# DmitryUlyanov/deep-image-prior

Hardware: AMD Instinct MI355X
Metric: optimisation iters/sec per image (skip-net 512x512 denoising) (higher is better)
Workload: dtype f32

## Files before the change

__graft_entry__.py:

```python
import os
import subprocess
import sys

ROOT = os.path.dirname(os.path.abspath(__file__))
PKG = os.path.join(ROOT, "deep-image-prior_amd")
CSRC = os.path.join(PKG, "csrc")
LIB = os.path.join(PKG, "lib", "libdip_hip.so")
SOURCES = ["dip_core.hip", "dip_list.hip", "conv_igemm.hip", "conv_igemm_dma.hip", "conv_small.hip", "conv_thin.hip", "conv_bf3.hip", "conv1x1_res.hip", "conv_thin4.hip", "conv_wgrad.hip", "wgrad_bf3.hip", "wgrad_tail.hip", "wgrad_thin.hip", "bn_kernels.hip", "bn_bwd_one.hip",
           "upcat_kernels.hip", "res_kernels.hip", "misc_kernels.hip", "monitor_kernels.hip", "loss_kernels.hip"]


def add_to_path():
    if PKG not in sys.path:
        sys.path.insert(0, PKG)
    return PKG


def source_id() -> str:
    import glob
    import hashlib
    h = hashlib.sha256()
    files = sorted(glob.glob(os.path.join(CSRC, "*.hip")) + glob.glob(os.path.join(CSRC, "*.h"))) + \
        [os.path.join(ROOT, "include", "dip_hip.h")]
    for f in files:
        h.update(os.path.basename(f).encode() + b"\0")
        with open(f, "rb") as fh:
            h.update(fh.read())
        h.update(b"\0")
    return h.hexdigest()[:16]


def library_id(path: str = LIB):
    try:
        with open(path, "rb") as fh:
            blob = fh.read()
    except OSError:
        return None
    k = blob.find(b"DIP_BUILD_ID=")
    if k < 0:
        return None
    end = blob.find(b"\0", k)
    return blob[k + 13:end].decode(errors="replace")


def _stale() -> bool:
    return library_id() != source_id()


def build(force: bool = False) -> None:
    hipcc = os.environ.get("HIPCC", "/opt/rocm/bin/hipcc")
    import fcntl
    os.makedirs(os.path.dirname(LIB), exist_ok=True)
    lock = open(os.path.join(os.path.dirname(LIB), ".build.lock"), "w")
    fcntl.flock(lock, fcntl.LOCK_EX)
    try:
        _build_locked(hipcc, force)
    finally:
        fcntl.flock(lock, fcntl.LOCK_UN)
        lock.close()
    add_to_path()
    import dip_native
    L = dip_native.lib()
    assert L.dip_abi_version() == dip_native.ABI_VERSION
    import models
    import utils.common_utils
    sys.path.insert(0, os.path.join(ROOT, "oracle"))
    import dip_oracle
    bid = L.dip_build_id().decode()
    if os.path.exists(hipcc) and bid != source_id():
        if library_id() == source_id():
            raise RuntimeError(f"libdip_hip.so was rebuilt (sources {source_id()}) but this process still has build {bid} "
                               "mapped: restart the process")
        raise RuntimeError(f"libdip_hip.so on disk is build {library_id()}, the sources are {source_id()}: the build recipe did "
                           "not produce a current library")
    print(f"[build] ok: {len(dip_native.EXPORTS)} C-ABI symbols, package importable, library built from sources {bid}"
          + ("" if bid == source_id() else f" (sources on disk: {source_id()}; no hipcc here to rebuild)"))


def _build_locked(hipcc: str, force: bool) -> None:
    if force or _stale():
        if not os.path.exists(hipcc):
            if os.path.exists(LIB):
                print(f"[build] {hipcc} not found; keeping the prebuilt {LIB}")
            else:
                raise RuntimeError(f"{hipcc} not found and {LIB} is not prebuilt")
        else:
            os.makedirs(os.path.join(CSRC, "build"), exist_ok=True)
            os.makedirs(os.path.dirname(LIB), exist_ok=True)
            sid = source_id()
            flags = ["--offload-arch=gfx950", "-O3", "-std=c++17", "-fPIC", "-I" + os.path.join(ROOT, "include"),
                     f'-DDIP_BUILD_ID="{sid}"']
            procs, objs = [], []
            import glob
            import hashlib
            hdr = hashlib.sha256()
            for f in sorted(glob.glob(os.path.join(CSRC, "*.h"))) + [os.path.join(ROOT, "include", "dip_hip.h")]:
                hdr.update(open(f, "rb").read())
            try:
                ver = subprocess.run([hipcc, "--version"], capture_output=True, timeout=60).stdout
            except Exception:
                ver = b"?"
            hdr.update(hipcc.encode() + b"\0" + ver)
            for s in SOURCES:
                fl = flags if s == "dip_core.hip" else flags[:-1]
                key = hashlib.sha256(hdr.digest() + open(os.path.join(CSRC, s), "rb").read() + " ".join(fl).encode()).hexdigest()[:12]
                o = os.path.join(CSRC, "build", s.replace(".hip", f".{key}.o"))
                objs.append(o)
                if not os.path.exists(o):
                    for stale in glob.glob(os.path.join(CSRC, "build", s.replace(".hip", ".*o"))):
                        os.remove(stale)
                    procs.append((s, o, subprocess.Popen([hipcc, *fl, "-c", os.path.join(CSRC, s), "-o", o + ".tmp.o"])))
            for s, o, p in procs:
                if p.wait() != 0:
                    raise RuntimeError(f"hipcc failed on {s}")
                os.replace(o + ".tmp.o", o)
            tmp = LIB + ".tmp"
            subprocess.check_call([hipcc, "--offload-arch=gfx950", "-shared", "-fPIC", *objs, "-o", tmp])
            os.replace(tmp, LIB)
            print(f"[build] built {LIB} from sources {sid}")


def smoke() -> None:
    import numpy as np
    import torch
    build()
    sys.path.insert(0, os.path.join(ROOT, "oracle"))
    import dip_oracle as O
    from models import get_net
    from utils.common_utils import get_noise, get_params, optimize
    assert torch.cuda.is_available(), "smoke() needs cuda:0 (MI355X)"
    dev = torch.device("cuda:0")
    torch.manual_seed(0)
    net = get_net(32, 'skip', 'reflection', skip_n33d=128, skip_n33u=128, skip_n11=4, num_scales=5,
                  upsample_mode='bilinear')
    sd = {k: v.detach().clone() for k, v in net.state_dict().items()
          if not k.endswith(("running_mean", "running_var", "num_batches_tracked"))}
    z = get_noise(32, 'noise', (128, 128))
    target = torch.rand(1, 3, 128, 128)
    spec = O.default_spec()

    def oracle(dt, masks=None, zrec=None):
        onet = O.OracleNet(spec, {k: v.to(dt) for k, v in sd.items()})
        o = onet(z.to(dt), None, masks, zrec)
        l = torch.nn.functional.mse_loss(o, target.to(dt))
        l.backward()
        return o.detach(), l.item(), {k: p.grad.detach().double() for k, p in zip(onet.names, onet.params)}

    zrec = {}
    out64, loss64, g64n = oracle(torch.float64, zrec=zrec)
    out_o, loss_o, g32 = oracle(torch.float32)
    net = net.to(dev)
    zg, tg = z.to(dev), target.to(dev)
    mse = torch.nn.MSELoss()
    rec = {}

    def closure():
        out = net(zg)
        loss = mse(out, tg)
        loss.backward()
        rec["out"], rec["loss"] = out.detach(), loss.detach()
        rec["grads"] = {k: p.grad.detach().clone() for k, p in net.named_parameters()}
        return loss

    optimize('adam', get_params('net', net, zg), closure, 0.01, 1)
    torch.cuda.synchronize()
    sys.path.insert(0, os.path.join(ROOT, "tests"))
    import hipops
    import parity
    hmasks = hipops.lrelu_masks(net, spec)
    _, _, g64 = oracle(torch.float64, hmasks)
    out = rec["out"].cpu()
    psnr = O.psnr(out.numpy(), out_o.numpy())
    rel = abs(rec["loss"].item() - loss_o) / abs(loss_o)
    rep = parity.grad_report(rec["grads"], g64, g32, g64n, parity.zero_grad_keys(spec, sd))
    mrep = parity.mask_report(hmasks, zrec)
    import ctypes as C
    import dip_native as N
    eng = net.__dict__["_dip_engine"]
    nb3 = sum(1 for fn, args, name in list(eng.fwd_ops) + list(eng.bwd_ops)
              if fn is eng.lib.dip_conv_igemm and eng.lib.dip_conv_bf3_eligible(args[0]))
    nw3 = sum(1 for fn, args, name in list(eng.bwd_ops) if fn is eng.lib.dip_conv_wgrad and eng.lib.dip_wgrad_bf3_eligible(args[0]))
    assert nb3 >= 1 and nw3 >= 1, f"smoke(): the bf16-pipe kernels are not on this launch list (conv_bf3 {nb3}, wgrad_bf3 {nw3})"
    print(f"[smoke] launches on the bf16 matrix pipe: conv_bf3 {nb3}, wgrad_bf3 {nw3}")
    print(f"[smoke] out PSNR vs oracle {psnr:.1f} dB, loss rel err {rel:.2e}, {parity.fmt(rep)}; {parity.fmt_masks(mrep)}")
    assert psnr > 100.0 and rel < 1e-5, (psnr, rel)
    parity.check(rep, mrep)
    print("[smoke] ok")


if __name__ == "__main__":
    cmd = sys.argv[1] if len(sys.argv) > 1 else "build"
    {"build": build, "smoke": smoke, "rebuild": lambda: build(True)}[cmd]()
```

deep-image-prior_amd/csrc/dip_gradsrc.h:

```cpp
#pragma once
#include "dip_common.h"

__device__ __forceinline__ f32x4 ld4(const float* p) { return *reinterpret_cast<const f32x4*>(p); }
__device__ __forceinline__ void st4(float* p, f32x4 v) { *reinterpret_cast<f32x4*>(p) = v; }

struct GradSrcThin {
    f32x4 w[4];
};
__device__ __forceinline__ GradSrcThin grad_src_thin(const DipGradSrc& s, int ch) {
    GradSrcThin t;
#pragma unroll
    for (int j = 0; j < 4; ++j) t.w[j] = (s.tw != nullptr && j < s.tn) ? ld4(s.tw + (size_t)j * s.tcw + ch) : f32x4{0.f, 0.f, 0.f, 0.f};
    return t;
}
__device__ __forceinline__ f32x4 grad_src_thin4(const DipGradSrc& s, const GradSrcThin& t, int r, int c, int W) {
    f32x4 gv = ld4(s.g + ((size_t)r * W + c) * s.Cg);
#pragma unroll
    for (int j = 1; j < 4; ++j) gv[j] = j < s.tn ? gv[j] : 0.f;
    f32x4 du;
#pragma unroll
    for (int e = 0; e < 4; ++e) du[e] = fmaf(gv[3], t.w[3][e], fmaf(gv[2], t.w[2][e], fmaf(gv[1], t.w[1][e], gv[0] * t.w[0][e])));
    return du;
}

__device__ __forceinline__ f32x4 grad_src4(const DipGradSrc& s, int r, int c, int H, int W, int ch) {
    if (s.tw != nullptr) return grad_src_thin4(s, grad_src_thin(s, ch), r, c, W);
    const int P = s.pad;
    const float* base = s.g + s.choff + ch;
    if (s.win_h > 0) {
        const int wr = r - s.win_y, wc = c - s.win_x;
        if (wr < 0 || wr >= s.win_h || wc < 0 || wc >= s.win_w) return f32x4{0.f, 0.f, 0.f, 0.f};
        return ld4(base + ((size_t)wr * s.win_w + wc) * s.Cg);
    }
    const int Wg = W + 2 * P;
    if (!s.fold || P == 0) return ld4(base + ((size_t)(r + P) * Wg + (c + P)) * s.Cg);
    if (s.fold == 2) {
        const int r0 = r == 0 ? 0 : r + P, r1 = r == H - 1 ? H - 1 + 2 * P : r + P;
        const int c0 = c == 0 ? 0 : c + P, c1 = c == W - 1 ? W - 1 + 2 * P : c + P;
        f32x4 acc = f32x4{0.f, 0.f, 0.f, 0.f};
        for (int i = r0; i <= r1; ++i)
            for (int j = c0; j <= c1; ++j) acc += ld4(base + ((size_t)i * Wg + j) * s.Cg);
        return acc;
    }
    int rr[3], nr = 0, cc[3], ncn = 0;
    rr[nr++] = r + P;
    if (r >= 1 && r <= P) rr[nr++] = P - r;
    if (r <= H - 2 && r >= H - 1 - P) rr[nr++] = 2 * (H - 1) - r + P;
    cc[ncn++] = c + P;
    if (c >= 1 && c <= P) cc[ncn++] = P - c;
    if (c <= W - 2 && c >= W - 1 - P) cc[ncn++] = 2 * (W - 1) - c + P;
    f32x4 acc = f32x4{0.f, 0.f, 0.f, 0.f};
    for (int i = 0; i < nr; ++i)
        for (int j = 0; j < ncn; ++j) acc += ld4(base + ((size_t)rr[i] * Wg + cc[j]) * s.Cg);
    return acc;
}

__device__ __forceinline__ f32x4 up_adj_du4(const float* base, int Cs_cat, int H, int W, int Hl, int Wl, int ody, int odx,
                                            int mode, int i, int j) {
    f32x4 du = f32x4{0.f, 0.f, 0.f, 0.f};
    if (mode == DIP_UP_NEAREST) {
#pragma unroll
        for (int dr = 0; dr < 2; ++dr)
#pragma unroll
            for (int dc = 0; dc < 2; ++dc) {
                const int hr = 2 * i + dr - ody, hc = 2 * j + dc - odx;
                const f32x4 gq = ld4(base + ((size_t)min(max(hr, 0), H - 1) * W + min(max(hc, 0), W - 1)) * Cs_cat);
                const float wq = (hr >= 0 && hr < H && hc >= 0 && hc < W) ? 1.f : 0.f;
#pragma unroll
                for (int e = 0; e < 4; ++e) du[e] = fmaf(wq, gq[e], du[e]);
            }
        return du;
    }
    auto inw = [](int u, int o, int nwin) { return (u - o >= 0 && u - o < nwin) ? 1.f : 0.f; };
    const float wr[4] = {(i >= 1 ? 0.25f : 0.f) * inw(2 * i - 1, ody, H), (i == 0 ? 1.f : 0.75f) * inw(2 * i, ody, H),
                         (i == Hl - 1 ? 1.f : 0.75f) * inw(2 * i + 1, ody, H),
                         (i + 1 <= Hl - 1 ? 0.25f : 0.f) * inw(2 * i + 2, ody, H)};
    const float wc[4] = {(j >= 1 ? 0.25f : 0.f) * inw(2 * j - 1, odx, W), (j == 0 ? 1.f : 0.75f) * inw(2 * j, odx, W),
                         (j == Wl - 1 ? 1.f : 0.75f) * inw(2 * j + 1, odx, W),
                         (j + 1 <= Wl - 1 ? 0.25f : 0.f) * inw(2 * j + 2, odx, W)};
    f32x4 gw[16];
#pragma unroll
    for (int tr = 0; tr < 4; ++tr) {
        const int hr = min(max(2 * i - 1 + tr - ody, 0), H - 1);
#pragma unroll
        for (int tc = 0; tc < 4; ++tc) {
            const int hc = min(max(2 * j - 1 + tc - odx, 0), W - 1);
            gw[tr * 4 + tc] = ld4(base + ((size_t)hr * W + hc) * Cs_cat);
        }
    }
#pragma unroll
    for (int tr = 0; tr < 4; ++tr)
#pragma unroll
        for (int tc = 0; tc < 4; ++tc) {
            const float w = wr[tr] * wc[tc];
#pragma unroll
            for (int e = 0; e < 4; ++e) du[e] = fmaf(w, gw[tr * 4 + tc][e], du[e]);
        }
    return du;
}

__device__ __forceinline__ f32x4 grad_src4(const DipGradSrc& s, const GradSrcThin& t, int r, int c, int H, int W, int ch) {
    if (s.tw != nullptr) return grad_src_thin4(s, t, r, c, W);
    return grad_src4(s, r, c, H, W, ch);
}
```

deep-image-prior_amd/csrc/dip_list.hip:

```cpp
#include "dip_common.h"
#include <string.h>
#include <utility>

namespace {

template <class T>
inline T slot_as(const uint64_t* s) {
    T v;
    memcpy(&v, s, sizeof(T));
    return v;
}
template <class... A, size_t... I>
inline int call_slots(int (*fn)(A...), const uint64_t* s, std::index_sequence<I...>) {
    return fn(slot_as<A>(s + I)...);
}
template <auto Fn> struct Thunk;
template <class... A, int (*Fn)(A...)>
struct Thunk<Fn> {
    static constexpr int nargs = (int)sizeof...(A);
    static int call(const uint64_t* s) { return call_slots(Fn, s, std::index_sequence_for<A...>{}); }
};

struct Entry {
    const char* name;
    int (*call)(const uint64_t*);
    int nargs;
};
#define DIP_REG(f) {#f, &Thunk<&f>::call, Thunk<&f>::nargs}
const Entry g_fns[] = {
    DIP_REG(dip_nchw_to_nhwc), DIP_REG(dip_nhwc_to_nchw), DIP_REG(dip_head_fwd), DIP_REG(dip_head_bwd),
    DIP_REG(dip_pack_weights), DIP_REG(dip_pack_weights_bf3),
    DIP_REG(dip_conv_igemm), DIP_REG(dip_conv_thin4), DIP_REG(dip_conv_igemm_dma_cols), DIP_REG(dip_conv_small), DIP_REG(dip_conv_thin),
    DIP_REG(dip_conv_dgrad_ring), DIP_REG(dip_conv_bf3_cols), DIP_REG(dip_conv_splitk_finish),
    DIP_REG(dip_conv_wgrad), DIP_REG(dip_wgrad_bf3), DIP_REG(dip_wgrad_thin), DIP_REG(dip_conv_wgrad_tail), DIP_REG(dip_wgrad_tail_stream), DIP_REG(dip_wgrad_reduce),
    DIP_REG(dip_bn_finalize), DIP_REG(dip_bn_bwd_stats), DIP_REG(dip_bn_bwd_stats_fin), DIP_REG(dip_bn_bwd_finalize),
    DIP_REG(dip_bn_bwd_finalize2), DIP_REG(dip_bn_bwd_apply), DIP_REG(dip_bn_bwd_apply_src), DIP_REG(dip_bn_bwd_apply_fin),
    DIP_REG(dip_bn_bwd_apply_src_fin), DIP_REG(dip_bn_bwd_one), DIP_REG(dip_fold_to_nchw), DIP_REG(dip_fold_to_nhwc),
    DIP_REG(dip_upcat_fwd), DIP_REG(dip_upcat_fwd_fin), DIP_REG(dip_avgpool2_fwd), DIP_REG(dip_avgpool2_bwd),
    DIP_REG(dip_maxpool2_fwd), DIP_REG(dip_maxpool2_bwd), DIP_REG(dip_upsample_bwd_stats), DIP_REG(dip_upsample_bwd_stats_crop),
    DIP_REG(dip_upsample_bwd_stats_crop_fin), DIP_REG(dip_upsample_bwd_one),
    DIP_REG(dip_adam_step), DIP_REG(dip_noise_axpy), DIP_REG(dip_adam_tick), DIP_REG(dip_adam_step_dev),
    DIP_REG(dip_noise_axpy_dev), DIP_REG(dip_noise_axpy_dev2), DIP_REG(dip_counter_add), DIP_REG(dip_counter_add_n),
    DIP_REG(dip_loss_head_fwd), DIP_REG(dip_loss_head_bwd), DIP_REG(dip_fit_monitor), DIP_REG(dip_fit_monitor_dev), DIP_REG(dip_arena_backtrack),
    DIP_REG(dip_lanczos_down_fwd), DIP_REG(dip_lanczos_down_bwd), DIP_REG(dip_down_dense_fwd), DIP_REG(dip_down_dense_bwd_data),
    DIP_REG(dip_down_dense_bwd_weight), DIP_REG(dip_res_join_fwd), DIP_REG(dip_res_join_bwd),
};
constexpr int NFN = (int)(sizeof(g_fns) / sizeof(g_fns[0]));

}

extern "C" int dip_list_fn_id(const char* name) {
    if (name == nullptr) return -1;
    for (int i = 0; i < NFN; ++i)
        if (strcmp(g_fns[i].name, name) == 0) return i;
    return -1;
}

extern "C" int dip_list_fn_nargs(int fn) { return (fn >= 0 && fn < NFN) ? g_fns[fn].nargs : -1; }

extern "C" int dip_list_run(const DipCmd* cmds, int n, void* const* streams, int nstreams, void* const* events, int nevents,
                            int* failed_at) {
    if (failed_at != nullptr) *failed_at = -1;
    for (int i = 0; i < n; ++i) {
        const DipCmd& c = cmds[i];
        int rc = 0;
        if (c.stream < 0 || c.stream >= nstreams) rc = -1;
        else if (c.kind == DIP_CMD_LAUNCH) {
            if (c.fn < 0 || c.fn >= NFN || c.slots == nullptr || c.nslots != g_fns[c.fn].nargs) rc = -1;
            else {
                c.slots[c.nslots - 1] = (uint64_t)reinterpret_cast<uintptr_t>(streams[c.stream]);
                rc = g_fns[c.fn].call(c.slots);
            }
        } else if (c.event < 0 || c.event >= nevents) rc = -1;
        else if (c.kind == DIP_CMD_RECORD)
            rc = (int)hipEventRecord(reinterpret_cast<hipEvent_t>(events[c.event]), reinterpret_cast<hipStream_t>(streams[c.stream]));
        else if (c.kind == DIP_CMD_WAIT)
            rc = (int)hipStreamWaitEvent(reinterpret_cast<hipStream_t>(streams[c.stream]), reinterpret_cast<hipEvent_t>(events[c.event]), 0);
        else rc = -1;
        if (rc != 0) {
            if (failed_at != nullptr) *failed_at = i;
            if (rc == -1 && c.kind != DIP_CMD_LAUNCH) dip_set_error("list_run: malformed command (stream / event index, kind)");
            else if (rc == -1 && (c.fn < 0 || c.fn >= NFN || c.slots == nullptr || c.nslots != g_fns[c.fn < 0 || c.fn >= NFN ? 0 : c.fn].nargs))
                dip_set_error("list_run: malformed LAUNCH command (function id, slot count)");
            else if (c.kind != DIP_CMD_LAUNCH) dip_set_error(hipGetErrorString((hipError_t)rc));
            return rc;
        }
    }
    return 0;
}

extern "C" int dip_iter_run(const DipPhase* phases, int nphases, void* const* streams, int nstreams, int* failed_at) {
    if (failed_at != nullptr) failed_at[0] = failed_at[1] = -1;
    if (phases == nullptr || nphases < 0 || streams == nullptr || nstreams < 1) {
        dip_set_error("iter_run: needs a phase table and at least one stream");
        return -1;
    }
    for (int p = 0; p < nphases; ++p) {
        const DipPhase& ph = phases[p];
        int at = -1;
        int rc = -1;
        if (ph.n < 0 || (ph.n > 0 && ph.cmds == nullptr) || ph.nevents < 0 || (ph.nevents > 0 && ph.events == nullptr))
            dip_set_error("iter_run: malformed phase (command / event table)");
        else rc = dip_list_run(ph.cmds, ph.n, streams, nstreams, ph.events, ph.nevents, &at);
        if (rc != 0) {
            if (failed_at != nullptr) { failed_at[0] = p; failed_at[1] = at; }
            return rc;
        }
    }
    return 0;
}

extern "C" int dip_events_create(void** events, int n) {
    for (int i = 0; i < n; ++i) {
        hipEvent_t e;
        hipError_t rc = hipEventCreateWithFlags(&e, hipEventDisableTiming);
        if (rc != hipSuccess) {
            dip_set_error(hipGetErrorString(rc));
            for (int j = 0; j < i; ++j) (void)hipEventDestroy(reinterpret_cast<hipEvent_t>(events[j]));
            return (int)rc;
        }
        events[i] = reinterpret_cast<void*>(e);
    }
    return 0;
}

extern "C" int dip_events_destroy(void** events, int n) {
    int rc = 0;
    for (int i = 0; i < n; ++i)
        if (events[i] != nullptr) {
            hipError_t e = hipEventDestroy(reinterpret_cast<hipEvent_t>(events[i]));
            if (e != hipSuccess) rc = (int)e;
            events[i] = nullptr;
        }
    return rc;
}
```

deep-image-prior_amd/dip_engine.py:

```python
from __future__ import annotations

import ctypes as C
import os
from typing import List, Optional

import torch

import dip_native as N
from dip_native import round_up


def _ptr(t: Optional[torch.Tensor], off_floats: int = 0) -> Optional[int]:
    if t is None:
        return None
    return t.data_ptr() + 4 * off_floats


class BNRec:

    def __init__(self, module: torch.nn.BatchNorm2d, name: str):
        self.module = module
        self.name = name
        self.C = module.num_features
        self.Cs = round_up(self.C, 4)
        self.gamma_off = self.beta_off = -1
        self.rm_off = self.rv_off = -1
        self.state = None
        self.coef = None


class ConvRec:
    def __init__(self, module: torch.nn.Conv2d, pad_mode: int, name: str):
        self.module = module
        self.name = name
        self.Cin, self.Cout = module.in_channels, module.out_channels
        self.ks = module.kernel_size[0]
        self.stride = module.stride[0]
        self.P = (self.ks - 1) // 2
        self.pad_mode = pad_mode if self.P > 0 else N.PAD_ZERO
        self.w_off = self.b_off = -1
        self.fwd_off = self.dgrad_off = -1
        self.need_dgrad = True

    @property
    def fwd_elems(self):
        return self.ks * self.ks * round_up(self.Cin, 4) * round_up(self.Cout, 32)

    @property
    def dgrad_elems(self):
        return self.ks * self.ks * round_up(self.Cout, 4) * round_up(self.Cin, 32)


class Act:

    def __init__(self, buf, H, W, Cch, bn: Optional[BNRec] = None, slope: float = 1.0):
        self.buf, self.H, self.W, self.C = buf, H, W, Cch
        self.Cs = round_up(Cch, 4)
        self.bn, self.slope = bn, slope

    def transform(self, shape_only=False) -> N.DipTransform:
        if self.bn is None:
            return N.DipTransform(None, None, 1.0)
        if shape_only:
            return N.DipTransform(1, 1, self.slope)
        assert self.bn.Cs == self.Cs
        return N.DipTransform(_ptr(self.bn.state, 2 * self.Cs), _ptr(self.bn.state, 3 * self.Cs), self.slope)


class ScalePlan:

    def __init__(self):
        self.skip_conv = self.skip_bn = None
        self.down_a = self.down_a_bn = self.down_b = self.down_b_bn = None
        self.cat_bn = self.up = self.up_bn = self.up1 = self.up1_bn = None
        self.ns = 0
        self.upsample_mode = "nearest"
        self.pool = None
        self.down_ds = None


class SkipEngine:
    kind = "skip"

    def __init__(self, net, scales: List[ScalePlan], out_conv: torch.nn.Conv2d, need_sigmoid: bool, pad: str,
                 act_slope: float = 0.2):
        self._init_common(net, need_sigmoid, pad, act_slope)
        self._collect_records(scales, out_conv)
        self.param_list = list(net.parameters())
        self._check_supported()

    def _init_common(self, net, need_sigmoid: bool, pad: str, act_slope: float):
        self.net = net
        self.need_sigmoid = need_sigmoid
        self.pad_mode = N.PAD_REFLECT if pad == "reflection" else N.PAD_ZERO
        self.slope = act_slope
        self.fwd_id = 0
        self._aux = {}
        self.two_streams = os.environ.get("DIP_TWO_STREAMS", "1") != "0"
        self.defer_scale = int(os.environ.get("DIP_DEFER_WGRAD", "2")) if self.two_streams else -1
        self.side_min_pixels = int(os.environ.get("DIP_SIDE_MIN_PIXELS", "0"))
        self._fwd_side, self._deferred, self._entered_defer_scale, self._fused_bnb = set(), [], False, {}
        self.use_clist = os.environ.get("DIP_NO_CLIST") is None
        import re
        ko = os.environ.get("DIP_KNOCKOUT")
        self._knockout = re.compile(ko) if ko else None
        self._ko_after, self._ko_seen = int(os.environ.get("DIP_KNOCKOUT_AFTER", "0")), {}
        self._clists = {}
        self._replicate_bufs = set()
        self.fuse_bnb = os.environ.get("DIP_BNB_FUSE", "0") == "1"
        self.fuse_bnb_1x1 = os.environ.get("DIP_BNB_FUSE", "0") == "2"
        self.thin_src = os.environ.get("DIP_NO_THIN_SRC") is None
        self.use_small = os.environ.get("DIP_CONV_NO_SMALL") is None
        self.ticket_fin = os.environ.get("DIP_TICKET_FIN") == "1"
        self.bnb_one = os.environ.get("DIP_BNB_NO_ONE") is None
        self.tail_inline = self.two_streams and os.environ.get("DIP_TAIL_INLINE", "1") != "0"
        self.bnb_fin_fuse = os.environ.get("DIP_BNB_FIN_FUSE") == "1"
        self.bulk2_max_pixels = 0
        if self.two_streams:
            env = os.environ.get("DIP_BULK2_MAX_PIXELS")
            self.bulk2_max_pixels = int(env) if env is not None else -1
        self._bulk2, self._bulk_flip = set(), False
        self.bf3 = False
        self.device = None
        self.shape_key = None
        self.lib = None
        self.slab = None

    def _collect_records(self, scales: List[ScalePlan], out_conv: torch.nn.Conv2d):
        self.nscales = len(scales)
        self.convs: List[ConvRec] = []
        self.bns: List[BNRec] = []
        self.sc = []
        for i, s in enumerate(scales):
            rec = ScalePlan()
            rec.ns, rec.upsample_mode = s.ns, s.upsample_mode
            rec.pool = getattr(s, 'pool', None)
            for attr in ("skip_conv", "down_a", "down_ds", "down_b", "up", "up1"):
                m = getattr(s, attr, None)
                if m is not None:
                    r = ConvRec(m, self.pad_mode, f"s{i}.{attr}")
                    if attr == "down_ds":
                        r.P = (r.ks - r.stride) // 2
                        r.pad_mode = N.PAD_REPLICATE
                    self.convs.append(r)
                    setattr(rec, attr, r)
            for attr in ("skip_bn", "down_a_bn", "down_b_bn", "cat_bn", "up_bn", "up1_bn"):
                m = getattr(s, attr)
                if m is not None:
                    r = BNRec(m, f"s{i}.{attr}")
                    self.bns.append(r)
                    setattr(rec, attr, r)
            self.sc.append(rec)
        self.out_conv = ConvRec(out_conv, self.pad_mode, "out")
        self.convs.append(self.out_conv)

    def _check_supported(self):
        for r in self.convs:
            lanczos_ds = r.name.endswith(".down_ds") and r.ks in (8, 12) and r.stride == 2
            if not lanczos_ds and (r.ks not in (1, 3, 5, 7) or r.stride not in (1, 2) or (r.ks == 1 and r.stride != 1)):
                raise NotImplementedError(f"dip-amd: conv {r.name} k={r.ks} s={r.stride} has no gfx950 kernel")
            m = r.module
            if m.dilation != (1, 1) or m.groups != 1 or m.kernel_size[0] != m.kernel_size[1]:
                raise NotImplementedError(f"dip-amd: conv {r.name}: dilation/groups/non-square unsupported")
        for b in self.bns:
            if b.module.momentum is None:
                raise NotImplementedError(f"dip-amd: BatchNorm {b.name}: momentum=None (cumulative moving average of "
                                          "the running statistics) is not implemented; the reference uses 0.1")
            if not b.module.affine:
                raise NotImplementedError(f"dip-amd: BatchNorm {b.name}: affine=False is not implemented")
        for i, s in enumerate(self.sc):
            if s.ns % 4 or s.down_b.Cout % 4 or s.up.Cout % 4 or (s.up.Cin % 4):
                raise NotImplementedError("dip-amd: internal channel counts must be multiples of 4")

    def _dalloc(self, n, dtype=torch.float32, zero=False):
        if self.slab is not None:
            return self.slab.alloc(int(n), dtype, zero)
        return (torch.zeros if zero else torch.empty)(int(n), dtype=dtype, device=self.device)

    def _dcopy(self, host_bytes):
        src = torch.frombuffer(bytearray(host_bytes), dtype=torch.uint8)
        t = self._dalloc(src.numel(), torch.uint8)
        t.copy_(src)
        return t

    def _build_arenas(self, device):
        self.lib = N.lib()
        self.device = device
        params = self.param_list
        off = 0
        slots = []
        for p in params:
            slots.append(off)
            off += round_up(p.numel(), 4)
        self.n_arena = off
        self.params = self._dalloc(off, zero=True)
        self.grads = self._dalloc(off, zero=True)
        self.slots = slots
        with torch.no_grad():
            for p, o in zip(params, slots):
                n = p.numel()
                self.params[o:o + n].copy_(p.detach().reshape(-1).to(device=device, dtype=torch.float32))
                p.data = self.params[o:o + n].view(p.shape)
        pid = {id(p): o for p, o in zip(params, slots)}
        for r in self.convs:
            r.w_off = pid[id(r.module.weight)]
            r.b_off = pid[id(r.module.bias)] if r.module.bias is not None else -1
        nb = sum(2 * b.Cs for b in self.bns)
        self.bnbuf = self._dalloc(max(nb, 4), zero=True)
        self.nbt = self._dalloc(max(len(self.bns), 1), torch.int64, zero=True)
        o = 0
        with torch.no_grad():
            for k, b in enumerate(self.bns):
                m = b.module
                b.gamma_off, b.beta_off = pid[id(m.weight)], pid[id(m.bias)]
                if m.track_running_stats and m.running_mean is not None:
                    b.rm_off, b.rv_off = o, o + b.Cs
                    self.bnbuf[o:o + b.C].copy_(m.running_mean.to(device))
                    self.bnbuf[o + b.Cs:o + b.Cs + b.C].copy_(m.running_var.to(device))
                    m._buffers["running_mean"] = self.bnbuf[o:o + b.C]
                    m._buffers["running_var"] = self.bnbuf[o + b.Cs:o + b.Cs + b.C]
                    self.nbt[k] = m.num_batches_tracked.to(device)
                    m._buffers["num_batches_tracked"] = self.nbt[k]
                o += 2 * b.Cs
                b.state = self._dalloc(4 * b.Cs, zero=True)
                b.coef = self._dalloc(2 * b.Cs, zero=True)
        off = 0
        recs = (N.DipPackRec * len(self.convs))()
        max_elems = 0
        for k, r in enumerate(self.convs):
            r.fwd_off = off
            off += r.fwd_elems
            r.dgrad_off = off
            off += r.dgrad_elems
            recs[k] = N.DipPackRec(r.w_off, r.fwd_off, r.dgrad_off, r.Cout, r.Cin, r.ks, round_up(r.Cin, 4),
                                   round_up(r.Cout, 32), round_up(r.Cout, 4), round_up(r.Cin, 32))
            max_elems = max(max_elems, r.fwd_elems + r.dgrad_elems)
        self.packed = self._dalloc(off, zero=True)
        self.bf3 = bool(self.lib.dip_conv_bf3_terms())
        if self.bf3:
            off3, max3 = 0, 0
            recs3 = (N.DipPackRec3 * len(self.convs))()
            for k, r in enumerate(self.convs):
                r.fwd3_off = r.dgrad3_off = -1
                nchF, nchD = (round_up(r.Cin, 4) + 15) // 16, (round_up(r.Cout, 4) + 15) // 16
                CoutP, CinP = round_up(r.Cout, 32), round_up(r.Cin, 32)
                k1 = (os.environ.get("DIP_CONV_BF3_1X1") == "1" and r.ks == 1 and r.Cin % 16 == 0 and r.Cout % 16 == 0
                      and min(r.Cin, r.Cout) >= 128)
                if (r.ks == 3 or k1) and r.stride == 1 and not r.name.endswith(".down_ds"):
                    kk = r.ks * r.ks
                    r.fwd3_off = off3
                    off3 += kk * nchF * 3 * CoutP * 16
                    r.dgrad3_off = off3
                    off3 += kk * nchD * 3 * CinP * 16
                    max3 = max(max3, kk * 16 * (nchF * CoutP + nchD * CinP))
                recs3[k] = N.DipPackRec3(r.w_off, r.fwd3_off, r.dgrad3_off, r.Cout, r.Cin, r.ks, nchF, CoutP, nchD, CinP)
            self.packed3 = self._dalloc(max(off3, 8), torch.int16, zero=True)
            self.pack_recs3 = self._dcopy(bytes(recs3))
            self.pack_max3 = max3
        self.pack_recs = self._dcopy(bytes(recs))
        self.pack_max = max_elems
        self.shape_key = None

    def _arena_ok(self) -> bool:
        if self.device is None:
            return False
        base = self.params.data_ptr()
        for p, o in zip(self.param_list, self.slots):
            if p.data_ptr() != base + 4 * o:
                return False
        return True

    def _new(self, n):
        t = self._dalloc(n)
        self._alloc.append(t)
        return t

    def _reset_sizing(self):
        self.stat_need = self.wg_need = self.wgb_need = self.bwdp_need = self.ws_need = 4
        self.wg2_need = self.wgb2_need = 4
        self.stat2_need = self.ws2_need = 4
        self.bwdp2_need = 4
        self.bwdp3_need = 4
        self.ticket_need = 8

    def _build_plan(self, H, W, Cin_img):
        if min(H, W) < 2 ** self.nscales:
            raise NotImplementedError(f"dip-amd: input {H}x{W} is too small for {self.nscales} scales")
        self.H, self.W, self.Cimg = H, W, Cin_img
        self._clists = {}
        self._reset_sizing()
        self._alloc = []
        oc = self.out_conv
        self.n_out = oc.Cout
        if getattr(self, "_bulk2_auto", self.bulk2_max_pixels < 0):
            self._bulk2_auto = True
            big, h, w = False, H, W
            for sc in self.sc:
                hl, wl = ((h + 1) // 2, (w + 1) // 2) if sc.pool is None else (h // 2, w // 2)
                for r, px in ((sc.down_a, hl * wl), (sc.down_b, hl * wl), (sc.up, h * w), (sc.up1, h * w)):
                    if r is not None and r.ks >= 3 and r.Cin >= 96 and r.Cout >= 96 and px >= 65536:
                        big = True
                h, w = hl, wl
            self.bulk2_max_pixels = 0 if big else 100000
        for sizing in (True, False):
            self._begin_pass(sizing)
            self.x_nhwc = self._buf(H * W * round_up(Cin_img, 4))
            xin = Act(self.x_nhwc, H, W, Cin_img)
            last = self._plan_scale(0, xin, H, W)
            self.Hout, self.Wout = last.H, last.W
            self.y_out = self._buf(last.H * last.W * round_up(oc.Cout, 4))
            self._emit_conv_fwd(oc, last, self.y_out, None)
            self.dy_out = self._buf(last.H * last.W * round_up(oc.Cout, 4))
            pre = []
            self._emit_wgrad(oc, last, self.dy_out, pre, scale=0)
            if self._thin_src_ok(oc, last):
                du_last = (self.dy_out, 0, oc)
            else:
                du_last = self._emit_dgrad(oc, last, self.dy_out, pre, fuse_bn=True)
            dy_last = self._emit_bn_act_bwd(last, du_last, pre)
            self.dbg_top = {"du_last": du_last, "dy_last": dy_last, "last": last}
            self.last_act = last
            self.bwd_ops = pre + self._bwd_scale_ops(0, dy_last)
            self.bwd_ops += self._flush_deferred_wgrads()
        self.shape_key = (H, W, Cin_img)

    def _begin_pass(self, sizing: bool):
        self._sizing = sizing
        self.fwd_ops, self.bwd_ops, self.bwd_input_ops, self.keep = [], [], [], []
        if not sizing:
            self.stats_scratch = self._new(self.stat_need)
            self.bwd_scratch = self._new(self.bwdp_need)
            self.wg_scratch = self._new(self.wg_need)
            self.wgb_scratch = self._new(self.wgb_need)
            self.wg_scratch2 = self._new(self.wg2_need)
            self.wgb_scratch2 = self._new(self.wgb2_need)
            self.ws_scratch = self._new(self.ws_need)
            self.stats_scratch2 = self._new(self.stat2_need)
            self.ws_scratch2 = self._new(self.ws2_need)
            self.bwd_scratch2 = self._new(self.bwdp2_need)
            self.bwd_scratch3 = self._new(self.bwdp3_need)
            self.tickets = self._dalloc(self.ticket_need, torch.int32, zero=True)
            self._alloc.append(self.tickets)
        self._ticket_off = 0
        self._fused_bnb = {}
        self._deferred = []
        self._replicate_bufs = set()
        self._fwd_side = set()
        self._bulk2, self._bulk_flip = set(), False
        self._entered_defer_scale = False

    def _plan_scale(self, i, xin: Act, H, W):
        s = self.sc[i]
        st = {}
        Hl, Wl = ((H + 1) // 2, (W + 1) // 2) if s.pool is None else (H // 2, W // 2)
        if s.ns:
            st["s_y"] = self._buf(H * W * round_up(s.ns, 4))
            self._emit_conv_fwd(s.skip_conv, xin, st["s_y"], s.skip_bn)
            st["s_act"] = Act(st["s_y"], H, W, s.ns, s.skip_bn, self.slope)
        st["d1_y"] = self._buf(Hl * Wl * round_up(s.down_a.Cout, 4))
        if s.pool in ('avg', 'max'):
            st["d1_full"] = self._buf(H * W * round_up(s.down_a.Cout, 4))
            self._emit_conv_fwd(s.down_a, xin, st["d1_full"], None)
            self._emit_avgpool(st["d1_full"], H, W, s.down_a.Cout, st["d1_y"], s.down_a_bn, s.pool)
        elif s.pool == 'lanczos':
            st["d1_full"] = self._buf(H * W * round_up(s.down_a.Cout, 4))
            self._emit_conv_fwd(s.down_a, xin, st["d1_full"], None)
            st["d1_raw"] = Act(st["d1_full"], H, W, s.down_a.Cout)
            self._emit_conv_fwd(s.down_ds, st["d1_raw"], st["d1_y"], s.down_a_bn)
        else:
            self._emit_conv_fwd(s.down_a, xin, st["d1_y"], s.down_a_bn)
        d1 = Act(st["d1_y"], Hl, Wl, s.down_a.Cout, s.down_a_bn, self.slope)
        st["d2_y"] = self._buf(Hl * Wl * round_up(s.down_b.Cout, 4))
        self._emit_conv_fwd(s.down_b, d1, st["d2_y"], s.down_b_bn)
        d2 = Act(st["d2_y"], Hl, Wl, s.down_b.Cout, s.down_b_bn, self.slope)
        st["d1"], st["d2"] = d1, d2
        deep = d2
        if i < self.nscales - 1:
            deep = self._plan_scale(i + 1, d2, Hl, Wl)
        st["deep"] = deep
        ccat = s.ns + deep.C
        assert ccat == s.cat_bn.C == s.up.Cin, (ccat, s.cat_bn.C, s.up.Cin)
        Hu, Wu = 2 * deep.H, 2 * deep.W
        if s.ns:
            Ho, Wo = min(H, Hu), min(W, Wu)
        else:
            Ho, Wo = Hu, Wu
        geom = dict(Hs=H, Ws=W, os_y=(H - Ho) // 2 if s.ns else 0, os_x=(W - Wo) // 2 if s.ns else 0,
                    Hd=deep.H, Wd=deep.W, od_y=(Hu - Ho) // 2, od_x=(Wu - Wo) // 2)
        default = (not s.ns or (Ho, Wo) == (H, W)) and deep.H == (Ho + 1) // 2 and deep.W == (Wo + 1) // 2 \
            and geom["od_y"] == 0 and geom["od_x"] == 0
        st["geom"] = None if default else geom
        st["cat"] = self._buf(Ho * Wo * round_up(ccat, 4))
        self._emit_upcat(s, st.get("s_act"), deep, st["cat"], Ho, Wo, st["geom"])
        cat = Act(st["cat"], Ho, Wo, ccat, s.cat_bn, 1.0)
        st["cat_act"] = cat
        st["u_y"] = self._buf(Ho * Wo * round_up(s.up.Cout, 4))
        self._emit_conv_fwd(s.up, cat, st["u_y"], s.up_bn)
        u = Act(st["u_y"], Ho, Wo, s.up.Cout, s.up_bn, self.slope)
        st["u"] = u
        res = u
        if s.up1 is not None:
            st["u1_y"] = self._buf(Ho * Wo * round_up(s.up1.Cout, 4))
            self._emit_conv_fwd(s.up1, u, st["u1_y"], s.up1_bn)
            res = Act(st["u1_y"], Ho, Wo, s.up1.Cout, s.up1_bn, self.slope)
            st["u1"] = res
        st["xin"], st["H"], st["W"], st["Ho"], st["Wo"] = xin, H, W, Ho, Wo
        s.st = st
        return res

    def _buf(self, n):
        return None if self._sizing else self._new(n)

    def _ticket(self, n=8):
        if self._sizing:
            self.ticket_need += n
            return None
        off = self._ticket_off
        self._ticket_off += n
        assert self._ticket_off <= self.tickets.numel()
        return self.tickets.data_ptr() + 4 * off

    def _bn_fin(self, bn: BNRec, ticket) -> N.DipBnFin:
        m = bn.module
        return N.DipBnFin(_ptr(self.params, bn.gamma_off), _ptr(self.params, bn.beta_off), float(m.eps), float(m.momentum),
                          _ptr(bn.state), bn.Cs, bn.C,
                          _ptr(self.bnbuf, bn.rm_off) if bn.rm_off >= 0 else None,
                          _ptr(self.bnbuf, bn.rv_off) if bn.rv_off >= 0 else None, ticket)

    def _bnb_fin(self, bn: BNRec, npix, ticket) -> N.DipBnbFin:
        return N.DipBnbFin(_ptr(self.grads, bn.gamma_off), _ptr(self.grads, bn.beta_off), _ptr(bn.coef), bn.C, npix,
                           ticket)

    def _emit_bn_finalize(self, bn: BNRec, scratch, rows, cstride):
        m = bn.module
        args = (_ptr(scratch), rows, cstride, bn.C, _ptr(self.params, bn.gamma_off), _ptr(self.params, bn.beta_off),
                float(m.eps), float(m.momentum), _ptr(bn.state), bn.Cs,
                _ptr(self.bnbuf, bn.rm_off) if bn.rm_off >= 0 else None,
                _ptr(self.bnbuf, bn.rv_off) if bn.rv_off >= 0 else None)
        self.fwd_ops.append((self.lib.dip_bn_finalize, args, "bn_fin:" + bn.name))

    def _emit_conv_fwd(self, r: ConvRec, x: Act, y, bn: Optional[BNRec]):
        assert x.C == r.Cin, (r.name, x.C, r.Cin)
        Ho = (x.H + 2 * r.P - r.ks) // r.stride + 1
        Wo = (x.W + 2 * r.P - r.ks) // r.stride + 1
        Cy = round_up(r.Cout, 4)
        sizing = self._sizing
        d = N.DipConvDesc(_ptr(x.buf), x.H, x.W, x.Cs, round_up(x.C, 4), x.transform(sizing),
                          None if sizing else _ptr(self.packed, r.fwd_off),
                          _ptr(self.params, r.b_off) if (r.b_off >= 0 and not sizing) else None,
                          _ptr(y), Ho, Wo, Cy, r.Cout, 0, r.ks, r.stride, r.pad_mode, r.P, 1, 0, None, 1, None)
        small = self.use_small and bool(self.lib.dip_conv_small_eligible(C.byref(d)))
        if small:
            ksplit, ntiles, wsf = 1, self.lib.dip_conv_small_rows(C.byref(d)), 0
        else:
            bf3_ok = self.bf3 and getattr(r, "fwd3_off", -1) >= 0 and not (x.bn is not None and round_up(x.C, 4) > 512)
            plan = N.conv_plan if bf3_ok else N.conv_plan_fp32
            ksplit, ntiles, wsf = plan(Ho, Wo, round_up(x.C, 4), r.Cout, r.ks, r.stride)
        side = r.name.endswith("skip_conv") and Ho * Wo >= self.side_min_pixels and bn is not None
        if side:
            self._fwd_side.update(("conv_fwd:" + r.name, "bn_fin:" + bn.name))
        if sizing:
            if side:
                if bn is not None:
                    self.stat2_need = max(self.stat2_need, ntiles * 3 * round_up(r.Cout, 32))
                self.ws2_need = max(self.ws2_need, wsf)
            else:
                if bn is not None:
                    self.stat_need = max(self.stat_need, ntiles * 3 * round_up(r.Cout, 32))
                self.ws_need = max(self.ws_need, wsf)
            return
        stats_scratch = self.stats_scratch2 if side else self.stats_scratch
        ws_scratch = self.ws_scratch2 if side else self.ws_scratch
        d.stats = _ptr(stats_scratch) if bn is not None else None
        if self.bf3 and getattr(r, "fwd3_off", -1) >= 0:
            d.wp3 = self.packed3.data_ptr() + 2 * r.fwd3_off
        d.ksplit = ksplit
        d.ws = _ptr(ws_scratch) if ksplit > 1 else None
        self.keep.append(d)
        lib = self.lib
        self.fwd_ops.append((lib.dip_conv_small if small else lib.dip_conv_igemm, (C.byref(d),), "conv_fwd:" + r.name))
        if bn is not None:
            self._emit_bn_finalize(bn, stats_scratch, ntiles, round_up(r.Cout, 32))

    def _emit_avgpool(self, x, H, W, Cc, y, bn: BNRec, kind='avg'):
        Cs = round_up(Cc, 4)
        nblk = self.lib.dip_upcat_nblk(H // 2, W // 2, Cc)
        if self._sizing:
            self.stat_need = max(self.stat_need, nblk * 3 * Cs)
            return
        fn = self.lib.dip_maxpool2_fwd if kind == 'max' else self.lib.dip_avgpool2_fwd
        self.fwd_ops.append((fn, (_ptr(x), H, W, Cs, Cc, _ptr(y), Cs, _ptr(self.stats_scratch), nblk), "pool:" + bn.name))
        self._emit_bn_finalize(bn, self.stats_scratch, nblk, Cs)

    def _emit_upcat(self, s, s_act: Optional[Act], deep: Act, cat, H, W, geom=None):
        Ccat = s.ns + deep.C
        Cs_cat = round_up(Ccat, 4)
        nblk = self.lib.dip_upcat_nblk(H, W, Ccat)
        fin_ok = self.ticket_fin and bool(self.lib.dip_fin_rows_ok(nblk, Ccat))
        ticket = self._ticket() if fin_ok else None
        if self._sizing:
            self.stat_need = max(self.stat_need, nblk * 3 * Cs_cat)
            return
        mode = N.UP_BILINEAR if s.upsample_mode == "bilinear" else N.UP_NEAREST
        d = N.DipUpcatDesc(_ptr(s_act.buf) if s_act else None, s_act.Cs if s_act else 4, s.ns,
                           s_act.transform() if s_act else N.DipTransform(None, None, 1.0),
                           _ptr(deep.buf), deep.Cs, deep.C, deep.transform(), H, W, mode, _ptr(cat), Cs_cat,
                           _ptr(self.stats_scratch), nblk)
        if geom is not None:
            for k, v in geom.items():
                setattr(d, k, v)
        self.keep.append(d)
        if fin_ok:
            fin = self._bn_fin(s.cat_bn, ticket)
            self.keep.append(fin)
            self.fwd_ops.append((self.lib.dip_upcat_fwd_fin, (C.byref(d), C.byref(fin)), "upcat:" + s.cat_bn.name))
            return
        self.fwd_ops.append((self.lib.dip_upcat_fwd, (C.byref(d),), "upcat:" + s.cat_bn.name))
        self._emit_bn_finalize(s.cat_bn, self.stats_scratch, nblk, Cs_cat)

    def _flush_deferred_wgrads(self):
        ops, self._deferred = self._deferred, []
        return ops

    def _emit_wgrad(self, r: ConvRec, x: Act, dy, ops, scale=None):
        Ho = (x.H + 2 * r.P - r.ks) // r.stride + 1
        Wo = (x.W + 2 * r.P - r.ks) // r.stride + 1
        CinP, CoutP = round_up(r.Cin, 32), round_up(r.Cout, 32)
        nsplit, tap_groups, chan_block = N.wgrad_plan2(Ho, Wo, r.Cin, r.Cout, r.ks, r.stride)
        if scale is not None and self.defer_scale >= 0:
            ops = self._deferred
        slab = r.ks * r.ks * CinP * CoutP
        second = False
        if Ho * Wo <= self.bulk2_max_pixels:
            second = self._bulk_flip
            self._bulk_flip = not self._bulk_flip
        if self._sizing:
            if second:
                self.wg2_need = max(self.wg2_need, nsplit * slab)
                self.wgb2_need = max(self.wgb2_need, nsplit * CoutP)
            else:
                self.wg_need = max(self.wg_need, nsplit * slab)
                self.wgb_need = max(self.wgb_need, nsplit * CoutP)
            return
        has_b = r.b_off >= 0
        wg, wgb = (self.wg_scratch2, self.wgb_scratch2) if second else (self.wg_scratch, self.wgb_scratch)
        if second:
            self._bulk2.update(("wgrad:" + r.name, "wgred:" + r.name))
        d = N.DipWgradDesc(_ptr(x.buf), x.H, x.W, x.Cs, x.C, x.transform(), _ptr(dy), Ho, Wo,
                           round_up(r.Cout, 4), r.Cout, r.ks, r.stride, r.pad_mode, r.P,
                           _ptr(wg), _ptr(wgb) if has_b else None, nsplit, tap_groups,
                           chan_block)
        self.keep.append(d)
        ops.append((self.lib.dip_conv_wgrad, (C.byref(d),), "wgrad:" + r.name))
        ops.append((self.lib.dip_wgrad_reduce,
                    (_ptr(wg), _ptr(wgb) if has_b else None, nsplit, r.ks, r.Cin, r.Cout,
                     _ptr(self.grads, r.w_off), _ptr(self.grads, r.b_off) if has_b else None), "wgred:" + r.name))

    def _emit_dgrad(self, r: ConvRec, x: Act, dy, ops, accumulate_into=None, fuse_bn=False, need_pad=0):
        Ho = (x.H + 2 * r.P - r.ks) // r.stride + 1
        Wo = (x.W + 2 * r.P - r.ks) // r.stride + 1
        reflect = r.pad_mode in (N.PAD_REFLECT, N.PAD_REPLICATE) and r.P > 0
        pad = r.P if reflect else 0
        Hg, Wg = x.H + 2 * pad, x.W + 2 * pad
        off = (r.ks - 1) if reflect else (r.ks - 1 - r.P)
        Cg = x.Cs
        if accumulate_into is not None:
            gbuf, gpad = accumulate_into
            if pad > gpad or r.stride != 1:
                raise NotImplementedError(f"dip-amd: {r.name}: a skip filter larger than the down filter (with "
                                          "reflection padding) or a strided skip conv has no gfx950 path")
            if self._sizing:
                return accumulate_into
            o = gpad - pad
            Wg2 = x.W + 2 * gpad
            ybase = _ptr(gbuf, (o * Wg2 + o) * Cg)
            d = N.DipConvDesc(_ptr(dy), Ho, Wo, round_up(r.Cout, 4), round_up(r.Cout, 4),
                              N.DipTransform(None, None, 1.0), _ptr(self.packed, r.dgrad_off), None,
                              ybase, Hg, Wg, Cg, r.Cin, Wg2, r.ks, 1, N.PAD_ZERO, off, 1, 1, None)
            self.keep.append(d)
            small = self.use_small and bool(self.lib.dip_conv_small_eligible(C.byref(d)))
            ops.append((self.lib.dip_conv_small if small else self.lib.dip_conv_igemm, (C.byref(d),), "dgrad+:" + r.name))
            return accumulate_into
        ring = False
        if reflect and r.pad_mode == N.PAD_REFLECT and r.ks == 3 and r.stride == 1 and self.use_small and need_pad == 0:
            di = N.DipConvDesc(None, Ho, Wo, round_up(r.Cout, 4), round_up(r.Cout, 4), N.DipTransform(None, None, 1.0), None,
                               None, None, x.H, x.W, Cg, r.Cin, 0, r.ks, 1, N.PAD_ZERO, 1, 1, 0, None, 1, None)
            if self.lib.dip_conv_dgrad_ring_ok(C.byref(di)) and not self.lib.dip_conv_small_eligible(C.byref(di)):
                ring, pad, Hg, Wg, off = True, 0, x.H, x.W, 1
        gbuf = self._buf(Hg * Wg * Cg)
        if r.stride == 2:
            ksplit, _, wsf = N.conv_plan_dil2(Hg, Wg, round_up(r.Cout, 4), r.Cin, r.ks)
        else:
            fuse_here = self.fuse_bnb or (self.fuse_bnb_1x1 and r.ks == 1 and r.stride == 1)
            bf3_ok = self.bf3 and getattr(r, "dgrad3_off", -1) >= 0 and not (fuse_bn and fuse_here and not ring and x.bn is not None)
            ksplit, _, wsf = (N.conv_plan if bf3_ok else N.conv_plan_fp32)(Hg, Wg, round_up(r.Cout, 4), r.Cin, r.ks, 1)
        sizing = self._sizing
        d = N.DipConvDesc(None if sizing else _ptr(dy), Ho, Wo, round_up(r.Cout, 4), round_up(r.Cout, 4),
                          N.DipTransform(None, None, 1.0), None if sizing else _ptr(self.packed, r.dgrad_off), None,
                          None if sizing else _ptr(gbuf), Hg, Wg, Cg, r.Cin, 0, r.ks, 1, N.PAD_ZERO, off, r.stride, 0, None,
                          ksplit, (None if sizing else _ptr(self.ws_scratch)) if ksplit > 1 else None)
        if self.bf3 and not sizing and getattr(r, "dgrad3_off", -1) >= 0:
            d.wp3 = self.packed3.data_ptr() + 2 * r.dgrad3_off
        small = self.use_small and bool(self.lib.dip_conv_small_eligible(C.byref(d)))
        if small:
            d.ksplit, d.ws = 1, None
            rows = self.lib.dip_conv_small_rows(C.byref(d))
            fuse = fuse_bn and x.bn is not None and r.pad_mode != N.PAD_REPLICATE and not self._bnb_one_ok(x)
            if sizing:
                if fuse:
                    self.bwdp_need = max(self.bwdp_need, rows * 2 * x.bn.Cs)
                return (gbuf, pad)
            if r.pad_mode == N.PAD_REPLICATE:
                self._replicate_bufs.add(gbuf.data_ptr())
            if fuse:
                bn = x.bn
                d.bnb_y, d.bnb_state = _ptr(x.buf), _ptr(bn.state)
                d.bnb_partials = _ptr(self.bwd_scratch)
                d.bnb_Cy, d.bnb_Cs, d.bnb_pad, d.bnb_slope = x.Cs, bn.Cs, pad, float(x.slope)
                self._fused_bnb[gbuf.data_ptr()] = (rows, 0, 0)
            self.keep.append(d)
            ops.append((self.lib.dip_conv_small, (C.byref(d),), "dgrad:" + r.name))
            return (gbuf, pad)
        variant = self.lib.dip_conv_variant(C.byref(d))
        fused = None
        fuse_here = self.fuse_bnb or (self.fuse_bnb_1x1 and r.ks == 1 and r.stride == 1)
        if fuse_bn and fuse_here and not ring and x.bn is not None and self.lib.dip_conv_bnb_fusable(C.byref(d)):
            bn = x.bn
            rows = self.lib.dip_conv_ntiles(Hg, Wg)
            c_lo = (r.Cin - 128) if variant == 3 else 0
            rows_lo = self.lib.dip_conv_thin4_ntiles(Hg, Wg) if c_lo else 0
            if c_lo % 4 == 0:
                fused = (rows, rows_lo, c_lo)
                self.bwdp_need = max(self.bwdp_need, rows * 2 * bn.Cs)
                self.bwdp3_need = max(self.bwdp3_need, rows_lo * 2 * bn.Cs)
        if sizing:
            self.ws_need = max(self.ws_need, wsf)
            return (gbuf, pad)
        if r.pad_mode == N.PAD_REPLICATE:
            self._replicate_bufs.add(gbuf.data_ptr())
        if fused is not None:
            bn = x.bn
            d.bnb_y, d.bnb_state = _ptr(x.buf), _ptr(bn.state)
            d.bnb_partials = _ptr(self.bwd_scratch)
            d.bnb_partials_thin = _ptr(self.bwd_scratch3) if fused[2] else None
            d.bnb_Cy, d.bnb_Cs, d.bnb_pad, d.bnb_slope = x.Cs, bn.Cs, pad, float(x.slope)
            self._fused_bnb[gbuf.data_ptr()] = fused
        self.keep.append(d)
        if variant == 3 and self.two_streams:
            ncols = r.Cin - 128
            ops.append((self.lib.dip_conv_thin4, (C.byref(d), ncols), "dgthin:" + r.name))
            ops.append((self.lib.dip_conv_igemm_dma_cols, (C.byref(d), ncols), "dgrad:" + r.name))
        else:
            ops.append((self.lib.dip_conv_igemm, (C.byref(d),), "dgrad:" + r.name))
        if ring:
            dr = N.DipConvDesc.from_buffer_copy(d)
            dr.ksplit, dr.ws = 1, None
            self.keep.append(dr)
            ops.append((self.lib.dip_conv_dgrad_ring, (C.byref(dr),), "dgring:" + r.name))
        return (gbuf, pad)

    def _thin_src_ok(self, oc: ConvRec, last: Act) -> bool:
        return (self.thin_src and oc.ks == 1 and oc.stride == 1 and oc.Cout <= 4 and oc.Cin % 4 == 0 and last.bn is not None
                and not self.fuse_bnb and not self._bnb_one_ok(last))

    def _gradsrc(self, g, Cg, choff=0, window=None):
        if len(g) == 3:
            buf, _, oc = g
            d = N.DipGradSrc(_ptr(buf), 0, 0, round_up(oc.Cout, 4), 0)
            d.tw, d.tn, d.tcw = _ptr(self.params, oc.w_off), oc.Cout, oc.Cin
            self.keep.append(d)
            return d
        buf, pad = g
        fold = 0 if pad == 0 else (2 if buf.data_ptr() in self._replicate_bufs else 1)
        d = N.DipGradSrc(_ptr(buf), pad, fold, Cg, choff)
        if window is not None:
            d.win_y, d.win_x, d.win_h, d.win_w = window
        self.keep.append(d)
        return d

    def _emit_bn_act_bwd(self, a: Act, g, ops, choff=0, Cg=None, side=False, window=None):
        bn = a.bn
        nblk = self.lib.dip_bn_bwd_nblk(a.H, a.W, a.C)
        fin_ok = self.ticket_fin and bool(self.lib.dip_fin_rows_ok(nblk, a.C))
        ticket = self._ticket() if fin_ok else None
        if self._sizing:
            if side:
                self.bwdp2_need = max(self.bwdp2_need, nblk * 2 * a.Cs)
            else:
                self.bwdp_need = max(self.bwdp_need, nblk * 2 * a.Cs)
            return None
        scratch = self.bwd_scratch2 if side else self.bwd_scratch
        dz = self._new(a.H * a.W * a.Cs)
        src = self._gradsrc(g, Cg if Cg is not None else a.Cs, choff, window)
        lib = self.lib
        if self._bnb_one_ok(a) and self._fused_bnb.get(g[0].data_ptr()) is None:
            ops.append((lib.dip_bn_bwd_one, (C.byref(src), _ptr(a.buf), a.H, a.W, a.Cs, a.C, _ptr(bn.state), bn.Cs,
                                             float(a.slope), _ptr(dz), a.Cs, _ptr(self.grads, bn.gamma_off),
                                             _ptr(self.grads, bn.beta_off), _ptr(bn.coef)), "bnb_one:" + bn.name))
            return dz
        fused = self._fused_bnb.get(g[0].data_ptr()) if (choff == 0 and not side) else None
        if fused is None and fin_ok:
            fin = self._bnb_fin(bn, a.H * a.W, ticket)
            self.keep.append(fin)
            ops.append((lib.dip_bn_bwd_stats_fin, (C.byref(src), _ptr(a.buf), a.H, a.W, a.Cs, a.C, _ptr(bn.state), bn.Cs,
                                                   float(a.slope), None, a.Cs, _ptr(scratch), nblk, C.byref(fin)),
                        "bnb_stats:" + bn.name))
        elif fused is not None:
            rows, rows_lo, c_lo = fused
            if c_lo == 0 and self._fin_rows_ok(rows, a.C):
                ops.append(self._apply_src_fin(src, a, bn, self.bwd_scratch, rows, dz))
                return dz
            ops.append((lib.dip_bn_bwd_finalize2, (_ptr(self.bwd_scratch), rows, _ptr(self.bwd_scratch3) if c_lo else None,
                                                   rows_lo, c_lo, bn.Cs, bn.C, a.H * a.W,
                                                   _ptr(self.grads, bn.gamma_off), _ptr(self.grads, bn.beta_off),
                                                   _ptr(bn.coef)), "bnb_fin:" + bn.name))
        else:
            ops.append((lib.dip_bn_bwd_stats, (C.byref(src), _ptr(a.buf), a.H, a.W, a.Cs, a.C, _ptr(bn.state), bn.Cs,
                                               float(a.slope), None, a.Cs, _ptr(scratch), nblk),
                        "bnb_stats:" + bn.name))
            if self._fin_rows_ok(nblk, a.C):
                ops.append(self._apply_src_fin(src, a, bn, scratch, nblk, dz))
                return dz
            ops.append((lib.dip_bn_bwd_finalize, (_ptr(scratch), nblk, bn.Cs, bn.C, a.H * a.W,
                                                  _ptr(self.grads, bn.gamma_off), _ptr(self.grads, bn.beta_off),
                                                  _ptr(bn.coef)), "bnb_fin:" + bn.name))
        ops.append((lib.dip_bn_bwd_apply_src, (C.byref(src), _ptr(a.buf), a.H, a.W, a.Cs, a.C, _ptr(bn.state), bn.Cs,
                                               float(a.slope), _ptr(bn.coef), _ptr(dz), a.Cs), "bnb_apply:" + bn.name))
        return dz

    def _fin_rows_ok(self, rows, Cc) -> bool:
        return self.bnb_fin_fuse and bool(self.lib.dip_bn_bwd_fin_rows_ok(rows, Cc))

    def _apply_src_fin(self, src, a: Act, bn: BNRec, scratch, rows, dz):
        return (self.lib.dip_bn_bwd_apply_src_fin,
                (C.byref(src), _ptr(a.buf), a.H, a.W, a.Cs, a.C, _ptr(bn.state), bn.Cs, float(a.slope), _ptr(scratch), rows,
                 _ptr(self.grads, bn.gamma_off), _ptr(self.grads, bn.beta_off), _ptr(bn.coef), _ptr(dz), a.Cs),
                "bnb_apply:" + bn.name)

    def _bnb_one_ok(self, a: Act) -> bool:
        return self.bnb_one and a.bn is not None and bool(self.lib.dip_bn_bwd_one_ok(a.H * a.W, a.C))

    def _emit_up_bwd(self, deep: Act, dcat, Cs_cat, choff, H, W, mode, ops, geom=None):
        bn = deep.bn
        nblk = self.lib.dip_bn_bwd_nblk(deep.H, deep.W, deep.C)
        fin_ok = self.ticket_fin and bool(self.lib.dip_fin_rows_ok(nblk, deep.C))
        ticket = self._ticket() if fin_ok else None
        if self._sizing:
            self.bwdp_need = max(self.bwdp_need, nblk * 2 * deep.Cs)
            return None
        dz = self._new(deep.H * deep.W * deep.Cs)
        lib = self.lib
        m = N.UP_BILINEAR if mode == "bilinear" else N.UP_NEAREST
        if self._bnb_one_ok(deep):
            gm = geom if geom is not None else dict(Hd=(H + 1) // 2, Wd=(W + 1) // 2, od_y=0, od_x=0)
            ops.append((lib.dip_upsample_bwd_one,
                        (_ptr(dcat), Cs_cat, choff, H, W, gm["Hd"], gm["Wd"], gm["od_y"], gm["od_x"], m, _ptr(deep.buf),
                         deep.Cs, deep.C, _ptr(bn.state), bn.Cs, float(deep.slope), _ptr(dz), deep.Cs,
                         _ptr(self.grads, bn.gamma_off), _ptr(self.grads, bn.beta_off), _ptr(bn.coef)), "upb_one:" + bn.name))
            return dz
        if fin_ok:
            fin = self._bnb_fin(bn, deep.H * deep.W, ticket)
            self.keep.append(fin)
            gm = geom if geom is not None else dict(Hd=(H + 1) // 2, Wd=(W + 1) // 2, od_y=0, od_x=0)
            ops.append((lib.dip_upsample_bwd_stats_crop_fin,
                        (_ptr(dcat), Cs_cat, choff, H, W, gm["Hd"], gm["Wd"], gm["od_y"], gm["od_x"], m,
                         _ptr(deep.buf), deep.Cs, deep.C, _ptr(bn.state), bn.Cs, float(deep.slope), _ptr(dz), deep.Cs,
                         _ptr(self.bwd_scratch), nblk, C.byref(fin)), "upb_stats:" + bn.name))
            ops.append((lib.dip_bn_bwd_apply, (_ptr(dz), deep.Cs, _ptr(deep.buf), deep.Cs, deep.H * deep.W, deep.C,
                                               _ptr(bn.state), bn.Cs, _ptr(bn.coef)), "bnb_apply:" + bn.name))
            return dz
        if geom is None:
            ops.append((lib.dip_upsample_bwd_stats, (_ptr(dcat), Cs_cat, choff, H, W, m, _ptr(deep.buf), deep.Cs, deep.C,
                                                     _ptr(bn.state), bn.Cs, float(deep.slope), _ptr(dz), deep.Cs,
                                                     _ptr(self.bwd_scratch), nblk), "upb_stats:" + bn.name))
        else:
            ops.append((lib.dip_upsample_bwd_stats_crop,
                        (_ptr(dcat), Cs_cat, choff, H, W, geom["Hd"], geom["Wd"], geom["od_y"], geom["od_x"], m,
                         _ptr(deep.buf), deep.Cs, deep.C, _ptr(bn.state), bn.Cs, float(deep.slope), _ptr(dz), deep.Cs,
                         _ptr(self.bwd_scratch), nblk), "upb_stats:" + bn.name))
        if self._fin_rows_ok(nblk, deep.C):
            ops.append((lib.dip_bn_bwd_apply_fin, (_ptr(dz), deep.Cs, _ptr(deep.buf), deep.Cs, deep.H * deep.W, deep.C,
                                                   _ptr(bn.state), bn.Cs, _ptr(self.bwd_scratch), nblk,
                                                   _ptr(self.grads, bn.gamma_off), _ptr(self.grads, bn.beta_off),
                                                   _ptr(bn.coef)), "bnb_apply:" + bn.name))
            return dz
        ops.append((lib.dip_bn_bwd_finalize, (_ptr(self.bwd_scratch), nblk, bn.Cs, bn.C, deep.H * deep.W,
                                              _ptr(self.grads, bn.gamma_off), _ptr(self.grads, bn.beta_off),
                                              _ptr(bn.coef)), "bnb_fin:" + bn.name))
        ops.append((lib.dip_bn_bwd_apply, (_ptr(dz), deep.Cs, _ptr(deep.buf), deep.Cs, deep.H * deep.W, deep.C,
                                           _ptr(bn.state), bn.Cs, _ptr(bn.coef)), "bnb_apply:" + bn.name))
        return dz

    def _bwd_scale_ops(self, i, dy_last):
        s = self.sc[i]
        st = s.st
        ops = []
        if i == self.defer_scale:
            self._entered_defer_scale = True
            ops += self._flush_deferred_wgrads()
        H, W, xin = st["H"], st["W"], st["xin"]
        Ho, Wo, geom = st["Ho"], st["Wo"], st["geom"]
        if s.up1 is not None:
            self._emit_wgrad(s.up1, st["u"], dy_last, ops, scale=i)
            g = self._emit_dgrad(s.up1, st["u"], dy_last, ops, fuse_bn=True)
            dy_u = self._emit_bn_act_bwd(st["u"], g, ops)
        else:
            dy_u = dy_last
        cat = st["cat_act"]
        self._emit_wgrad(s.up, cat, dy_u, ops, scale=i)
        g = self._emit_dgrad(s.up, cat, dy_u, ops, fuse_bn=True)
        dcat = self._emit_bn_act_bwd(cat, g, ops)
        dy_s = None
        if s.ns:
            win = (geom["os_y"], geom["os_x"], Ho, Wo) if (geom is not None and (Ho, Wo) != (H, W)) else None
            dy_s = self._emit_bn_act_bwd(st["s_act"], (dcat, 0), ops, choff=0, Cg=cat.Cs, side=True, window=win)
            self._emit_wgrad(s.skip_conv, xin, dy_s, ops, scale=i)
        deep = st["deep"]
        dy_deep = self._emit_up_bwd(deep, dcat, cat.Cs, s.ns, Ho, Wo, s.upsample_mode, ops, geom)
        if self._entered_defer_scale:
            ops += self._flush_deferred_wgrads()
        if i < self.nscales - 1:
            ops += self._bwd_scale_ops(i + 1, dy_deep)
            gin = self.sc[i + 1].gin
            dy_d2 = self._emit_bn_act_bwd(st["d2"], gin, ops)
        else:
            dy_d2 = dy_deep
        inline_tail = i == 0 and self.tail_inline
        self._emit_wgrad(s.down_b, st["d1"], dy_d2, ops, scale=None if inline_tail else i)
        g = self._emit_dgrad(s.down_b, st["d1"], dy_d2, ops, fuse_bn=True)
        dy_d1 = self._emit_bn_act_bwd(st["d1"], g, ops)
        if s.pool == 'lanczos':
            Cs1 = round_up(s.down_a.Cout, 4)
            raw = st["d1_raw"]
            self._emit_wgrad(s.down_ds, raw, dy_d1, ops, scale=i)
            g2 = self._emit_dgrad(s.down_ds, raw, dy_d1, ops)
            dy_full = self._buf(H * W * Cs1)
            if not self._sizing:
                src = self._gradsrc(g2, Cs1)
                ops.append((self.lib.dip_fold_to_nhwc, (C.byref(src), H, W, s.down_a.Cout, _ptr(dy_full), Cs1),
                            "fold:" + s.down_ds.name))
            dy_d1 = dy_full
        if s.pool in ('avg', 'max'):
            Cs1 = round_up(s.down_a.Cout, 4)
            dy_full = self._buf(H * W * Cs1)
            if not self._sizing:
                if s.pool == 'avg':
                    ops.append((self.lib.dip_avgpool2_bwd, (_ptr(dy_d1), H, W, Cs1, s.down_a.Cout, _ptr(dy_full), Cs1),
                                "poolb:" + s.down_a_bn.name))
                else:
                    ops.append((self.lib.dip_maxpool2_bwd, (_ptr(dy_d1), _ptr(st["d1_full"]), H, W, Cs1, Cs1,
                                                            s.down_a.Cout, _ptr(dy_full), Cs1),
                                "poolb:" + s.down_a_bn.name))
            dy_d1 = dy_full
        self._emit_wgrad(s.down_a, xin, dy_d1, ops, scale=None if inline_tail else i)
        tgt = ops if i > 0 else self.bwd_input_ops
        sk = s.skip_conv if s.ns else None
        sk_pad = sk.P if (sk is not None and sk.P > 0 and sk.pad_mode in (N.PAD_REFLECT, N.PAD_REPLICATE)) else 0
        g = self._emit_dgrad(s.down_a, xin, dy_d1, tgt, need_pad=sk_pad)
        if s.ns:
            g = self._emit_dgrad(s.skip_conv, xin, dy_s, tgt, accumulate_into=g)
        s.gin = g
        if self._entered_defer_scale:
            ops += self._flush_deferred_wgrads()
        s.dbg = {"dy_last": dy_last, "dy_u": dy_u, "dcat": dcat, "dy_s": dy_s, "dy_deep": dy_deep, "dy_d2": dy_d2,
                 "dy_d1": dy_d1}
        return ops

    def _schedule(self, ops, cls_fn=None, join_before_fn=None, deps=None):
        sched = []
        if cls_fn is None:
            return [("launch", k, 0) for k in range(len(ops))]
        deps = deps or {}
        producers = {p for ps in deps.values() for p in ps}
        main_seq = 0
        forked = [0, -1, -1, -1]
        pending = [False, False, False, False]
        for k, (fn, args, name) in enumerate(ops):
            c = cls_fn(name)
            if c and forked[c] != main_seq:
                sched += [("record", ("fork", k), 0), ("wait", c, ("fork", k))]
                forked[c] = main_seq
            if c == 0 and pending[1] and join_before_fn(name):
                sched += [("record", ("join", k), 1), ("wait", 0, ("join", k))]
                pending[1] = False
            for prod in deps.get(name, ()):
                sched.append(("wait", c, ("dep", prod)))
            sched.append(("launch", k, c))
            if name in producers:
                sched.append(("record", ("dep", name), c))
            if c:
                pending[c] = True
            else:
                main_seq += 1
        for c in (1, 2, 3):
            if pending[c]:
                sched += [("record", ("join", -c), c), ("wait", 0, ("join", -c))]
        return sched

    def _aux_streams(self):
        slot = "cap" if torch.cuda.is_current_stream_capturing() else "eager"
        st_ = self._aux.get((slot, self.device))
        if st_ is None:
            st_ = self._aux[(slot, self.device)] = ([torch.cuda.Stream(self.device) for _ in range(3)], {})
        return slot, st_[0], st_[1]

    def _issue(self, ops, main, key, cls_fn=None, join_before_fn=None, deps=None, compile_only=False):
        multi = cls_fn is not None
        slot, aux, events = self._aux_streams() if multi else ("one", [], None)
        ko = False
        if self._knockout is not None:
            n = self._ko_seen[key] = self._ko_seen.get(key, 0) + 1
            ko = n > self._ko_after
        ck = (key, len(ops), multi, ko)
        ent = self._clists.get(ck)
        if ent is None:
            sched = self._schedule(ops, cls_fn, join_before_fn, deps)
            if ko:
                sched = [c for c in sched if not (c[0] == "launch" and self._knockout.search(ops[c[1]][2]))]
            cl = None
            if self.use_clist:
                evidx = {}
                cmds = []
                for c in sched:
                    if c[0] == "launch":
                        fn, args, name = ops[c[1]]
                        cmds.append(("launch", fn, args, c[2], name))
                    elif c[0] == "record":
                        cmds.append(("record", evidx.setdefault(c[1], len(evidx)), c[2]))
                    else:
                        cmds.append(("wait", c[1], evidx.setdefault(c[2], len(evidx))))
                cl = N.CmdList(cmds)
            ent = self._clists[ck] = (sched, cl)
        sched, cl = ent
        if compile_only:
            return cl
        if cl is not None:
            cl.run([main.cuda_stream] + [s_.cuda_stream for s_ in aux], slot)
            return
        streams = [main] + aux
        ptrs = [s_.cuda_stream for s_ in streams]
        check = N.check
        for c in sched:
            if c[0] == "launch":
                fn, args, name = ops[c[1]]
                rc = fn(*args, ptrs[c[2]])
                if rc:
                    check(rc, name)
            elif c[0] == "record":
                ev = events.get((key, c[1]))
                if ev is None:
                    ev = events[(key, c[1])] = torch.cuda.Event()
                ev.record(streams[c[2]])
            else:
                streams[c[1]].wait_event(events[(key, c[2])])

    def _run(self, ops, main, key="one", compile_only=False):
        return self._issue(ops, main, key, compile_only=compile_only)

    def _run_two_streams(self, ops, main, cls_fn, join_before_fn, key, deps=None, compile_only=False):
        return self._issue(ops, main, key, cls_fn, join_before_fn, deps, compile_only)

    _BWD_SIDE = staticmethod(lambda n: 2 if n.startswith(("wgrad:", "wgred:")) else
                             (1 if (n.startswith("dgthin:") or n.endswith(".skip_bn")) else 0))

    def _backward_deps(self, ops):
        names = [name for _, _, name in ops]
        present = set(names)
        deps = {}
        for i, sc in enumerate(self.sc):
            c, p = f"dgrad+:s{i}.skip_conv", f"bnb_apply:s{i}.skip_bn"
            if p not in present:
                p = f"bnb_one:s{i}.skip_bn"
            if sc.ns and c in present and p in present:
                deps.setdefault(c, []).append(p)
            c = f"wgrad:s{i}.skip_conv"
            if sc.ns and c in present and p in present:
                deps.setdefault(c, []).append(p)
        for k, name in enumerate(names):
            if not name.startswith("dgthin:"):
                continue
            main_part = "dgrad:" + name[len("dgthin:"):]
            j = names.index(main_part, k)
            consumer = next((n for n in names[j + 1:] if not self._BWD_SIDE(n)), None)
            if consumer is not None:
                deps.setdefault(consumer, []).append(name)
        return deps

    def _run_backward_two_streams(self, ops, main, compile_only=False):
        deps = self._bwd_deps if getattr(self, "_bwd_deps_for", None) is ops else None
        if deps is None:
            deps = self._bwd_deps = self._backward_deps(ops)
            self._bwd_deps_for = ops
        capturing = torch.cuda.is_current_stream_capturing()
        bulk2 = self._bulk2 if not capturing else ()
        cls = self._BWD_SIDE if not bulk2 else (lambda n: 3 if n in bulk2 else self._BWD_SIDE(n))
        return self._run_two_streams(ops, main, cls, lambda n: False, "bwd_cap" if capturing else "bwd", deps, compile_only)

    def _run_forward_two_streams(self, ops, main, compile_only=False):
        side = self._fwd_side
        return self._run_two_streams(ops, main, lambda n: 1 if n in side else 0, lambda n: n.startswith("upcat:"), "fwd",
                                     compile_only=compile_only)

    def _forward_prologue(self, x_ptr):
        lib = self.lib
        ops = [(lib.dip_pack_weights, (_ptr(self.params), _ptr(self.packed), self.pack_recs.data_ptr(),
                                       len(self.convs), self.pack_max), "pack_weights")]
        if self.bf3:
            ops.append((lib.dip_pack_weights_bf3, (_ptr(self.params), self.packed3.data_ptr(), self.pack_recs3.data_ptr(),
                                                   len(self.convs), self.pack_max3), "pack_weights_bf3"))
        ops.append((lib.dip_nchw_to_nhwc, (x_ptr, _ptr(self.x_nhwc), self.Cimg, self.H * self.W, round_up(self.Cimg, 4)),
                    "nchw_to_nhwc"))
        return ops

    def _launch_forward(self, x_ptr, main, with_out_conv=True, compile_only=False):
        if not compile_only:
            stream = main.cuda_stream
            for fn, args, name in self._forward_prologue(x_ptr):
                N.check(fn(*args, stream), name)
        ops = self.fwd_ops if with_out_conv else self.fwd_ops[:-1]
        if self.two_streams:
            return self._run_forward_two_streams(ops, main, compile_only)
        return self._run(ops, main, "fwd1", compile_only)

    def _launch_backward(self, main, compile_only=False):
        if self.two_streams:
            return self._run_backward_two_streams(self.bwd_ops, main, compile_only)
        return self._run(self.bwd_ops, main, "bwd1", compile_only)

    def iteration_lists(self):
        if not self.use_clist:
            raise RuntimeError("dip-amd: the native iteration chains compiled command lists; DIP_NO_CLIST=1 switches them off")
        if self._knockout is not None:
            raise RuntimeError("dip-amd: DIP_KNOCKOUT is a timing experiment of the eager path; the native iteration refuses it")
        if torch.cuda.is_current_stream_capturing():
            raise RuntimeError("dip-amd: the native iteration is an eager form; hipGraph capture goes through GraphedIteration")
        return self._launch_forward(None, None, False, compile_only=True), self._launch_backward(None, compile_only=True)

    def _net_cin(self) -> int:
        return self.sc[0].down_a.Cin

    def _input_gin(self):
        return self.sc[0].gin

    def forward(self, x: torch.Tensor, head=None):
        if x.dim() != 4 or x.shape[0] != 1:
            raise NotImplementedError("dip-amd: input must be [1,C,H,W] (train-mode BatchNorm couples a batch; "
                                      "independent images run as independent nets)")
        if not self.net.training:
            raise NotImplementedError("dip-amd: eval-mode BatchNorm is not implemented (the reference never "
                                      "calls .eval() on the skip path)")
        dev = x.device
        if self.device != dev or not self._arena_ok():
            self._build_arenas(dev)
        _, Cimg, H, W = x.shape
        if self.shape_key != (H, W, Cimg):
            if Cimg != self._net_cin():
                raise RuntimeError(f"dip-amd: input has {Cimg} channels, net expects {self._net_cin()}")
            self._build_plan(H, W, Cimg)
        lib = self.lib
        with torch.cuda.device(dev):
            main = torch.cuda.current_stream(dev)
            stream = main.cuda_stream
            xs = x.detach()
            if xs.dtype != torch.float32:
                xs = xs.float()
            xs = xs.contiguous()
            self.fwd_id += 1
            self._launch_forward(xs.data_ptr(), main, head is None)
            Ho_, Wo_ = self.Hout, self.Wout
            out = torch.empty((1, self.n_out, Ho_, Wo_), dtype=torch.float32, device=dev)
            loss = None
            if head is None:
                N.check(lib.dip_head_fwd(_ptr(self.y_out), out.data_ptr(), self.n_out, Ho_ * Wo_, round_up(self.n_out, 4),
                                         1 if self.need_sigmoid else 0, stream), "head_fwd")
            else:
                loss = torch.empty((), dtype=torch.float32, device=dev)
                self._head_desc = head._descriptor(self, out, loss)
                N.check(lib.dip_loss_head_fwd(C.byref(self._head_desc), stream), "loss_head_fwd")
            if len(self.bns):
                self.nbt.add_(1)
        self.last_out = out.detach()
        self.last_head = head
        return out if head is None else (loss, out)

    def _detach_stale_grads(self):
        base = self.grads.data_ptr()
        stale = [k for k, (p, o) in enumerate(zip(self.param_list, self.slots))
                 if p.grad is not None and p.grad.data_ptr() == base + 4 * o]
        if not stale:
            return
        if getattr(self, "grads_alt", None) is None or self.grads_alt.numel() != self.grads.numel() \
                or self.grads_alt.device != self.grads.device:
            self.grads_alt = torch.empty_like(self.grads)
        self.grads_alt.copy_(self.grads)
        for k in stale:
            p, o = self.param_list[k], self.slots[k]
            p.grad = self.grads_alt[o:o + p.numel()].view(p.shape)

    def backward(self, gout, fwd_id: int, need_input_grad: bool, gloss=None):
        if fwd_id != self.fwd_id:
            raise RuntimeError("dip-amd: backward() of a stale forward: the engine keeps the activations of the "
                               "most recent net(x) only (one forward, one backward per closure call)")
        dev = self.device
        lib = self.lib
        H, W = self.H, self.W
        grads = self.grads
        with torch.cuda.device(dev):
            main = torch.cuda.current_stream(dev)
            stream = main.cuda_stream
            self._detach_stale_grads()
            if self.last_head is None:
                g = gout.detach()
                if g.dtype != torch.float32:
                    g = g.float()
                g = g.contiguous()
                N.check(lib.dip_head_bwd(g.data_ptr(), self.last_out.data_ptr(), _ptr(self.dy_out), self.n_out,
                                         self.Hout * self.Wout,
                                         round_up(self.n_out, 4), 1 if self.need_sigmoid else 0, stream), "head_bwd")
            else:
                gl = gloss.detach().reshape(1)
                if gl.dtype != torch.float32:
                    gl = gl.float()
                self._gloss_keep = gl
                N.check(lib.dip_loss_head_bwd(C.byref(self._head_desc), gl.data_ptr(), _ptr(self.dy_out),
                                              round_up(self.n_out, 4), stream), "loss_head_bwd")
            self._launch_backward(main)
            gx = None
            if need_input_grad:
                self._run(self.bwd_input_ops, main, "bwdin")
                gbuf, pad = self._input_gin()
                src = N.DipGradSrc(_ptr(gbuf), pad, 1 if pad > 0 else 0, round_up(self.Cimg, 4), 0)
                gx = torch.empty((1, self.Cimg, H, W), dtype=torch.float32, device=dev)
                N.check(lib.dip_fold_to_nchw(C.byref(src), H, W, self.Cimg, gx.data_ptr(), stream), "fold_to_nchw")
        views = [grads[o:o + p.numel()].view(p.shape) for p, o in zip(self.param_list, self.slots)]
        return gx, views


class TableAct(Act):

    def __init__(self, buf, H, W, Cch, table, slope):
        super().__init__(buf, H, W, Cch, None, slope)
        self.table = table

    def transform(self, shape_only=False) -> N.DipTransform:
        if self.slope == 1.0:
            return N.DipTransform(None, None, 1.0)
        if shape_only:
            return N.DipTransform(1, 1, self.slope)
        return N.DipTransform(_ptr(self.table), _ptr(self.table, self.Cs), self.slope)


class ResBlockRec:

    def __init__(self, conv1, bn1, conv2, bn2):
        self.conv1, self.bn1, self.conv2, self.bn2 = conv1, bn1, conv2, bn2
        self.st = None


class ResNetEngine(SkipEngine):
    kind = "resnet"

    def __init__(self, net, first_conv, blocks, tail_conv, tail_bn, out_conv, need_residual: bool, pad: str,
                 act_slope: float = 0.2):
        self._init_common(net, True, pad, act_slope)
        self.defer_scale = -1
        self.nscales, self.sc = 0, []
        self.need_residual = bool(need_residual)
        self.first = ConvRec(first_conv, self.pad_mode, "first")
        self.blocks = []
        self.bns = []
        for k, (c1, b1, c2, b2) in enumerate(blocks):
            blk = ResBlockRec(ConvRec(c1, N.PAD_ZERO, f"b{k}.conv1"), BNRec(b1, f"b{k}.bn1"),
                              ConvRec(c2, N.PAD_ZERO, f"b{k}.conv2"), BNRec(b2, f"b{k}.bn2"))
            self.blocks.append(blk)
            self.bns += [blk.bn1, blk.bn2]
        self.tail = ConvRec(tail_conv, N.PAD_ZERO, "tail")
        self.tail_bn = BNRec(tail_bn, "tail_bn")
        self.bns.append(self.tail_bn)
        self.out_conv = ConvRec(out_conv, self.pad_mode, "out")
        self.convs = [self.first] + [c for b in self.blocks for c in (b.conv1, b.conv2)] + [self.tail, self.out_conv]
        self.param_list = list(net.parameters())
        self.gin = None
        self._check_supported()

    def _check_supported(self):
        super()._check_supported()
        if self.first.Cout % 4:
            raise NotImplementedError("dip-amd: internal channel counts must be multiples of 4")
        for r in self.convs:
            if r.ks != 3 or r.stride != 1:
                raise NotImplementedError(f"dip-amd: ResNet conv {r.name}: only 3x3 stride-1 convs are planned")
            if r is not self.first and r is not self.out_conv and tuple(r.module.padding) != (1, 1):
                raise NotImplementedError(f"dip-amd: ResNet conv {r.name}: padding {r.module.padding} (the join needs equal sizes)")

    def _net_cin(self) -> int:
        return self.first.Cin

    def _input_gin(self):
        return self.gin

    def _emit_join_fwd(self, xa: Act, xb: Act, out, name):
        if self._sizing:
            return
        ta, tb = xa.transform(), xb.transform()
        self.keep += [ta, tb]
        self.fwd_ops.append((self.lib.dip_res_join_fwd, (_ptr(xa.buf), xa.Cs, C.byref(ta), _ptr(xb.buf), xb.Cs, C.byref(tb),
                                                         _ptr(out), xa.Cs, xa.H * xa.W, xa.C), "res_join_fwd:" + name))

    def _emit_join_bwd(self, g, gd, a: Act, ops, name, act_of: Optional[Act] = None):
        if self._sizing:
            return (None, 0)
        out = self._new(a.H * a.W * a.Cs)
        src = self._gradsrc(gd, a.Cs)
        ty = None
        if act_of is not None:
            ty = act_of.transform()
            self.keep.append(ty)
        assert g is None or g[1] == 0
        ops.append((self.lib.dip_res_join_bwd, (_ptr(g[0]) if g is not None else None, a.Cs, C.byref(src),
                                                _ptr(act_of.buf) if act_of is not None else None, a.Cs,
                                                C.byref(ty) if ty is not None else None, _ptr(out), a.Cs, a.H, a.W, a.C), name))
        return (out, 0)

    def _build_plan(self, H, W, Cin_img):
        if min(H, W) < 2:
            raise NotImplementedError(f"dip-amd: input {H}x{W} is too small for a padded 3x3 convolution")
        self.H, self.W, self.Cimg = H, W, Cin_img
        self._clists = {}
        self._reset_sizing()
        self._alloc = []
        oc = self.out_conv
        self.n_out = oc.Cout
        if getattr(self, "_bulk2_auto", self.bulk2_max_pixels < 0):
            self._bulk2_auto = True
            big = any(r.Cin >= 96 and r.Cout >= 96 and H * W >= 65536 for r in self.convs)
            self.bulk2_max_pixels = 0 if big else 100000
        Cc = self.first.Cout
        n = H * W * round_up(Cc, 4)
        for sizing in (True, False):
            self._begin_pass(sizing)
            self.x_nhwc = self._buf(H * W * round_up(Cin_img, 4))
            xin = Act(self.x_nhwc, H, W, Cin_img)
            table = None
            if not sizing:
                Cs = round_up(Cc, 4)
                table = self._new(2 * Cs)
                table[:Cs] = 1.0
                table[Cs:] = 0.0
            c0 = self._buf(n)
            self._emit_conv_fwd(self.first, xin, c0, None)
            self.R0 = R0 = R = TableAct(c0, H, W, Cc, table, self.slope)
            for k, b in enumerate(self.blocks):
                c1, c2 = self._buf(n), self._buf(n)
                self._emit_conv_fwd(b.conv1, R, c1, b.bn1)
                A1 = Act(c1, H, W, Cc, b.bn1, self.slope)
                self._emit_conv_fwd(b.conv2, A1, c2, b.bn2)
                A2 = Act(c2, H, W, Cc, b.bn2, 1.0)
                b.st = (R, A1, A2)
                if self.need_residual:
                    r = self._buf(n)
                    self._emit_join_fwd(R, A2, r, f"b{k}")
                    R = Act(r, H, W, Cc)
                else:
                    R = A2
            ct = self._buf(n)
            self._emit_conv_fwd(self.tail, R, ct, self.tail_bn)
            T = Act(ct, H, W, Cc, self.tail_bn, 1.0)
            self.Hout, self.Wout = H, W
            self.y_out = self._buf(H * W * round_up(oc.Cout, 4))
            self._emit_conv_fwd(oc, T, self.y_out, None)
            self.dy_out = self._buf(H * W * round_up(oc.Cout, 4))
            ops = []
            self._emit_wgrad(oc, T, self.dy_out, ops)
            g = self._emit_dgrad(oc, T, self.dy_out, ops, fuse_bn=True)
            dy = self._emit_bn_act_bwd(T, g, ops)
            self._emit_wgrad(self.tail, R, dy, ops)
            G = self._emit_dgrad(self.tail, R, dy, ops, fuse_bn=R.bn is not None)
            for k in range(len(self.blocks) - 1, -1, -1):
                b = self.blocks[k]
                Rk, A1, A2 = b.st
                dy2 = self._emit_bn_act_bwd(A2, G, ops)
                self._emit_wgrad(b.conv2, A1, dy2, ops)
                g1 = self._emit_dgrad(b.conv2, A1, dy2, ops, fuse_bn=True)
                dy1 = self._emit_bn_act_bwd(A1, g1, ops)
                self._emit_wgrad(b.conv1, Rk, dy1, ops)
                gd = self._emit_dgrad(b.conv1, Rk, dy1, ops, fuse_bn=Rk.bn is not None)
                if self.need_residual:
                    G = self._emit_join_bwd(G, gd, Rk, ops, f"res_join_bwd:b{k}", act_of=R0 if k == 0 else None)
                else:
                    G = gd
            if not (self.need_residual and self.blocks):
                G = self._emit_join_bwd(None, G, R0, ops, "act_bwd:first", act_of=R0)
            dy0 = G[0]
            self._emit_wgrad(self.first, xin, dy0, ops)
            self.gin = self._emit_dgrad(self.first, xin, dy0, self.bwd_input_ops)
            self.last_act = T
            self.bwd_ops = ops
        self.shape_key = (H, W, Cin_img)

    def forward(self, x: torch.Tensor, head=None):
        if head is not None:
            raise NotImplementedError("dip-amd: the fused loss head (utils.loss_head.MSEHead) does not cover the ResNet backbone")
        if _graph_warmup[0] or (x.is_cuda and torch.cuda.is_current_stream_capturing()):
            raise NotImplementedError("dip-amd: hipGraph capture (GraphedIteration / optimize(graph=True)) is not implemented "
                                      "for the ResNet backbone; run it eagerly")
        return super().forward(x, head)


_graph_warmup = [0]


class _SkipFn(torch.autograd.Function):
    @staticmethod
    def forward(ctx, engine: SkipEngine, x, *params):
        out = engine.forward(x)
        ctx.engine = engine
        ctx.fwd_id = engine.fwd_id
        return out

    @staticmethod
    @torch.autograd.function.once_differentiable
    def backward(ctx, gout):
        need_x = ctx.needs_input_grad[1]
        gx, views = ctx.engine.backward(gout, ctx.fwd_id, need_x)
        return (None, gx, *views)


class _SkipLossFn(torch.autograd.Function):

    @staticmethod
    def forward(ctx, engine: SkipEngine, head, x, *params):
        loss, out = engine.forward(x, head)
        ctx.engine = engine
        ctx.fwd_id = engine.fwd_id
        ctx.mark_non_differentiable(out)
        return loss, out

    @staticmethod
    @torch.autograd.function.once_differentiable
    def backward(ctx, gloss, gout_unused):
        need_x = ctx.needs_input_grad[2]
        gx, views = ctx.engine.backward(None, ctx.fwd_id, need_x, gloss=gloss)
        return (None, None, gx, *views)


def _check_input(engine: SkipEngine, x: torch.Tensor):
    if not x.is_cuda:
        raise RuntimeError("dip-amd: the skip-net runs on an MI355X only (input tensor is on the CPU); there is "
                           "no CPU fallback in this backend")
    if engine.device != x.device or not engine._arena_ok():
        engine._build_arenas(x.device)


def run_net(engine: SkipEngine, x: torch.Tensor) -> torch.Tensor:
    _check_input(engine, x)
    return _SkipFn.apply(engine, x, *engine.param_list)


def run_net_loss(engine: SkipEngine, head, x: torch.Tensor):
    _check_input(engine, x)
    return _SkipLossFn.apply(engine, head, x, *engine.param_list)
```

deep-image-prior_amd/dip_native.py:

```python
from __future__ import annotations

import ctypes as C
import os

_HERE = os.path.dirname(os.path.abspath(__file__))
LIB_PATH = os.path.join(_HERE, "lib", "libdip_hip.so")
ABI_VERSION = 8

PAD_ZERO, PAD_REFLECT, PAD_REPLICATE = 0, 1, 2
UP_NEAREST, UP_BILINEAR = 0, 1

c_float_p = C.c_void_p


class DipTransform(C.Structure):
    _fields_ = [("a", C.c_void_p), ("b", C.c_void_p), ("slope", C.c_float)]


class DipPackRec(C.Structure):
    _fields_ = [("w_off", C.c_int64), ("fwd_off", C.c_int64), ("dgrad_off", C.c_int64),
                ("Cout", C.c_int32), ("Cin", C.c_int32), ("KS", C.c_int32),
                ("CinP4", C.c_int32), ("CoutP32", C.c_int32), ("CoutP4", C.c_int32), ("CinP32", C.c_int32)]


class DipPackRec3(C.Structure):
    _fields_ = [("w_off", C.c_int64), ("fwd_off", C.c_int64), ("dgrad_off", C.c_int64),
                ("Cout", C.c_int32), ("Cin", C.c_int32), ("KS", C.c_int32),
                ("nchF", C.c_int32), ("CoutP32", C.c_int32), ("nchD", C.c_int32), ("CinP32", C.c_int32)]


class DipBnFin(C.Structure):
    _fields_ = [("gamma", C.c_void_p), ("beta", C.c_void_p), ("eps", C.c_float), ("momentum", C.c_float),
                ("state", C.c_void_p), ("Cs", C.c_int32), ("C", C.c_int32), ("running_mean", C.c_void_p),
                ("running_var", C.c_void_p), ("ticket", C.c_void_p)]


class DipBnbFin(C.Structure):
    _fields_ = [("dgamma", C.c_void_p), ("dbeta", C.c_void_p), ("coef", C.c_void_p), ("C", C.c_int32),
                ("npix", C.c_int32), ("ticket", C.c_void_p)]


class DipConvDesc(C.Structure):
    _fields_ = [("x", C.c_void_p), ("Hin", C.c_int32), ("Win", C.c_int32), ("Cx", C.c_int32), ("Cin", C.c_int32),
                ("tr", DipTransform), ("wp", C.c_void_p), ("bias", C.c_void_p), ("y", C.c_void_p),
                ("Hout", C.c_int32), ("Wout", C.c_int32), ("Cy", C.c_int32), ("Cout", C.c_int32),
                ("y_pitch", C.c_int32),
                ("ks", C.c_int32), ("stride", C.c_int32), ("pad_mode", C.c_int32), ("off", C.c_int32),
                ("dil", C.c_int32), ("accumulate", C.c_int32), ("stats", C.c_void_p),
                ("ksplit", C.c_int32), ("ws", C.c_void_p),
                ("bnb_y", C.c_void_p), ("bnb_state", C.c_void_p), ("bnb_partials", C.c_void_p),
                ("bnb_partials_thin", C.c_void_p), ("bnb_Cy", C.c_int32), ("bnb_Cs", C.c_int32),
                ("bnb_pad", C.c_int32), ("bnb_slope", C.c_float),
                ("wp3", C.c_void_p)]


class DipWgradDesc(C.Structure):
    _fields_ = [("x", C.c_void_p), ("Hin", C.c_int32), ("Win", C.c_int32), ("Cx", C.c_int32), ("Cin", C.c_int32),
                ("tr", DipTransform), ("dy", C.c_void_p),
                ("Hout", C.c_int32), ("Wout", C.c_int32), ("Cdy", C.c_int32), ("Cout", C.c_int32),
                ("ks", C.c_int32), ("stride", C.c_int32), ("pad_mode", C.c_int32), ("off", C.c_int32),
                ("partial", C.c_void_p), ("bias_partial", C.c_void_p), ("nsplit", C.c_int32),
                ("tap_groups", C.c_int32), ("chan_block", C.c_int32)]


class DipGradSrc(C.Structure):
    _fields_ = [("g", C.c_void_p), ("pad", C.c_int32), ("fold", C.c_int32), ("Cg", C.c_int32), ("choff", C.c_int32),
                ("win_y", C.c_int32), ("win_x", C.c_int32), ("win_h", C.c_int32), ("win_w", C.c_int32),
                ("tw", C.c_void_p), ("tn", C.c_int32), ("tcw", C.c_int32)]


class DipUpcatDesc(C.Structure):
    _fields_ = [("s", C.c_void_p), ("Cs_s", C.c_int32), ("ns", C.c_int32), ("ts", DipTransform),
                ("d", C.c_void_p), ("Cs_d", C.c_int32), ("nd", C.c_int32), ("td", DipTransform),
                ("H", C.c_int32), ("W", C.c_int32), ("mode", C.c_int32),
                ("cat", C.c_void_p), ("Cs_cat", C.c_int32),
                ("stats", C.c_void_p), ("nblk", C.c_int32),
                ("Hs", C.c_int32), ("Ws", C.c_int32), ("os_y", C.c_int32), ("os_x", C.c_int32),
                ("Hd", C.c_int32), ("Wd", C.c_int32), ("od_y", C.c_int32), ("od_x", C.c_int32)]


class DipCmd(C.Structure):
    _fields_ = [("kind", C.c_int32), ("fn", C.c_int32), ("stream", C.c_int32), ("event", C.c_int32),
                ("slots", C.POINTER(C.c_uint64)), ("nslots", C.c_int32), ("reserved", C.c_int32)]


class DipPhase(C.Structure):
    _fields_ = [("cmds", C.POINTER(DipCmd)), ("events", C.POINTER(C.c_void_p)), ("n", C.c_int32), ("nevents", C.c_int32)]


class DipIterState(C.Structure):
    _fields_ = [("step", C.c_uint64), ("step_size", C.c_float), ("bc2_sqrt", C.c_float)]


class DipLossHeadDesc(C.Structure):
    _fields_ = [("u", C.c_void_p), ("Cu", C.c_int32), ("Cin", C.c_int32), ("tr", DipTransform),
                ("w", C.c_void_p), ("bias", C.c_void_p), ("Cout", C.c_int32), ("HW", C.c_int32),
                ("sigmoid", C.c_int32), ("target", C.c_void_p), ("mask", C.c_void_p), ("mask_c", C.c_int32),
                ("out", C.c_void_p), ("partials", C.c_void_p), ("nblk", C.c_int32), ("loss", C.c_void_p)]


class DipFitMonitorDesc(C.Structure):
    _fields_ = [("out", C.c_void_p), ("noisy", C.c_void_p), ("gt", C.c_void_p), ("out_avg", C.c_void_p), ("n", C.c_int64),
                ("exp_weight", C.c_float), ("backtrack_db", C.c_float), ("loss", C.c_void_p), ("partial", C.c_void_p),
                ("records", C.c_void_p), ("capacity", C.c_int32), ("show_every", C.c_int32), ("backtracking", C.c_int32),
                ("reserved", C.c_int32), ("counter", C.c_void_p), ("state", C.c_void_p)]


_SIGS = {
    "dip_abi_version": (C.c_int, []),
    "dip_build_id": (C.c_char_p, []),
    "dip_last_error": (C.c_char_p, []),
    "dip_device_pci_bus_id": (C.c_int, [C.c_int, C.c_char_p, C.c_int]),
    "dip_list_fn_id": (C.c_int, [C.c_char_p]),
    "dip_list_fn_nargs": (C.c_int, [C.c_int]),
    "dip_list_run": (C.c_int, [C.POINTER(DipCmd), C.c_int, C.POINTER(C.c_void_p), C.c_int, C.POINTER(C.c_void_p), C.c_int,
                               C.POINTER(C.c_int)]),
    "dip_iter_run": (C.c_int, [C.POINTER(DipPhase), C.c_int, C.POINTER(C.c_void_p), C.c_int, C.POINTER(C.c_int)]),
    "dip_events_create": (C.c_int, [C.POINTER(C.c_void_p), C.c_int]),
    "dip_events_destroy": (C.c_int, [C.POINTER(C.c_void_p), C.c_int]),
    "dip_nchw_to_nhwc": (C.c_int, [C.c_void_p, C.c_void_p, C.c_int, C.c_int, C.c_int, C.c_void_p]),
    "dip_nhwc_to_nchw": (C.c_int, [C.c_void_p, C.c_void_p, C.c_int, C.c_int, C.c_int, C.c_int, C.c_void_p]),
    "dip_head_fwd": (C.c_int, [C.c_void_p, C.c_void_p, C.c_int, C.c_int, C.c_int, C.c_int, C.c_void_p]),
    "dip_head_bwd": (C.c_int, [C.c_void_p, C.c_void_p, C.c_void_p, C.c_int, C.c_int, C.c_int, C.c_int, C.c_void_p]),
    "dip_pack_weights": (C.c_int, [C.c_void_p, C.c_void_p, C.c_void_p, C.c_int, C.c_int, C.c_void_p]),
    "dip_pack_weights_bf3": (C.c_int, [C.c_void_p, C.c_void_p, C.c_void_p, C.c_int, C.c_longlong, C.c_void_p]),
    "dip_conv_bf3_eligible": (C.c_int, [C.POINTER(DipConvDesc)]),
    "dip_conv_bf3_cols": (C.c_int, [C.POINTER(DipConvDesc), C.c_int, C.c_int, C.c_void_p]),
    "dip_conv_bf3_terms": (C.c_int, []),
    "dip_conv_bf3_set_terms": (C.c_int, [C.c_int]),
    "dip_conv_igemm": (C.c_int, [C.POINTER(DipConvDesc), C.c_void_p]),
    "dip_conv_ntiles": (C.c_int, [C.c_int, C.c_int]),
    "dip_conv_variant": (C.c_int, [C.POINTER(DipConvDesc)]),
    "dip_conv_bnb_fusable": (C.c_int, [C.POINTER(DipConvDesc)]),
    "dip_conv_thin4_ntiles": (C.c_int, [C.c_int, C.c_int]),
    "dip_conv_splitk_finish": (C.c_int, [C.POINTER(DipConvDesc), C.c_void_p]),
    "dip_conv_thin": (C.c_int, [C.POINTER(DipConvDesc), C.c_void_p]),
    "dip_conv_thin_eligible": (C.c_int, [C.POINTER(DipConvDesc)]),
    "dip_conv_thin_shape_ok": (C.c_int, [C.c_int, C.c_int, C.c_int, C.c_int, C.c_int, C.c_int]),
    "dip_conv_small": (C.c_int, [C.POINTER(DipConvDesc), C.c_void_p]),
    "dip_conv_small_eligible": (C.c_int, [C.POINTER(DipConvDesc)]),
    "dip_conv_small_rows": (C.c_int, [C.POINTER(DipConvDesc)]),
    "dip_conv_dgrad_ring": (C.c_int, [C.POINTER(DipConvDesc), C.c_void_p]),
    "dip_conv_dgrad_ring_ok": (C.c_int, [C.POINTER(DipConvDesc)]),
    "dip_conv_thin4": (C.c_int, [C.POINTER(DipConvDesc), C.c_int, C.c_void_p]),
    "dip_conv_igemm_dma_cols": (C.c_int, [C.POINTER(DipConvDesc), C.c_int, C.c_void_p]),
    "dip_conv_plan": (C.c_int, [C.c_int, C.c_int, C.c_int, C.c_int, C.c_int, C.c_int, C.POINTER(C.c_int),
                                C.POINTER(C.c_int), C.POINTER(C.c_int64)]),
    "dip_conv_plan_fp32": (C.c_int, [C.c_int, C.c_int, C.c_int, C.c_int, C.c_int, C.c_int, C.POINTER(C.c_int), C.POINTER(C.c_int),
                                    C.POINTER(C.c_int64)]),
    "dip_conv_plan_dil2": (C.c_int, [C.c_int, C.c_int, C.c_int, C.c_int, C.c_int, C.POINTER(C.c_int),
                                     C.POINTER(C.c_int), C.POINTER(C.c_int64)]),
    "dip_conv_wgrad": (C.c_int, [C.POINTER(DipWgradDesc), C.c_void_p]),
    "dip_wgrad_bf3_eligible": (C.c_int, [C.POINTER(DipWgradDesc)]),
    "dip_wgrad_bf3": (C.c_int, [C.POINTER(DipWgradDesc), C.c_void_p]),
    "dip_conv_wgrad_tail": (C.c_int, [C.POINTER(DipWgradDesc), C.c_void_p]),
    "dip_wgrad_tail_stream_ok": (C.c_int, [C.POINTER(DipWgradDesc)]),
    "dip_wgrad_tail_stream": (C.c_int, [C.POINTER(DipWgradDesc), C.c_void_p]),
    "dip_conv_wgrad_ntiles": (C.c_int, [C.c_int, C.c_int]),
    "dip_wgrad_thin": (C.c_int, [C.POINTER(DipWgradDesc), C.c_void_p]),
    "dip_wgrad_thin_eligible": (C.c_int, [C.POINTER(DipWgradDesc)]),
    "dip_wgrad_thin_shape_ok": (C.c_int, [C.c_int, C.c_int, C.c_int, C.c_int, C.c_int, C.c_int]),
    "dip_wgrad_thin_nsplit": (C.c_int, [C.c_int, C.c_int, C.c_int, C.c_int, C.c_int, C.c_int]),
    "dip_wgrad_plan": (C.c_int, [C.c_int, C.c_int, C.c_int, C.c_int, C.c_int, C.c_int, C.POINTER(C.c_int)]),
    "dip_wgrad_plan2": (C.c_int, [C.c_int, C.c_int, C.c_int, C.c_int, C.c_int, C.c_int, C.POINTER(C.c_int),
                                  C.POINTER(C.c_int), C.POINTER(C.c_int)]),
    "dip_wgrad_reduce": (C.c_int, [C.c_void_p, C.c_void_p, C.c_int, C.c_int, C.c_int, C.c_int, C.c_void_p,
                                   C.c_void_p, C.c_void_p]),
    "dip_bn_finalize": (C.c_int, [C.c_void_p, C.c_int, C.c_int, C.c_int, C.c_void_p, C.c_void_p, C.c_float,
                                  C.c_float, C.c_void_p, C.c_int, C.c_void_p, C.c_void_p, C.c_void_p]),
    "dip_bn_bwd_stats": (C.c_int, [C.POINTER(DipGradSrc), C.c_void_p, C.c_int, C.c_int, C.c_int, C.c_int,
                                   C.c_void_p, C.c_int, C.c_float, C.c_void_p, C.c_int, C.c_void_p, C.c_int,
                                   C.c_void_p]),
    "dip_bn_bwd_nblk": (C.c_int, [C.c_int, C.c_int, C.c_int]),
    "dip_bn_bwd_finalize": (C.c_int, [C.c_void_p, C.c_int, C.c_int, C.c_int, C.c_int, C.c_void_p, C.c_void_p,
                                      C.c_void_p, C.c_void_p]),
    "dip_bn_bwd_finalize2": (C.c_int, [C.c_void_p, C.c_int, C.c_void_p, C.c_int, C.c_int, C.c_int, C.c_int, C.c_int,
                                       C.c_void_p, C.c_void_p, C.c_void_p, C.c_void_p]),
    "dip_bn_bwd_apply": (C.c_int, [C.c_void_p, C.c_int, C.c_void_p, C.c_int, C.c_int, C.c_int, C.c_void_p, C.c_int,
                                   C.c_void_p, C.c_void_p]),
    "dip_bn_bwd_apply_src": (C.c_int, [C.POINTER(DipGradSrc), C.c_void_p, C.c_int, C.c_int, C.c_int, C.c_int,
                                       C.c_void_p, C.c_int, C.c_float, C.c_void_p, C.c_void_p, C.c_int, C.c_void_p]),
    "dip_bn_bwd_fin_rows_ok": (C.c_int, [C.c_int, C.c_int]),
    "dip_bn_bwd_apply_fin": (C.c_int, [C.c_void_p, C.c_int, C.c_void_p, C.c_int, C.c_int, C.c_int, C.c_void_p, C.c_int,
                                       C.c_void_p, C.c_int, C.c_void_p, C.c_void_p, C.c_void_p, C.c_void_p]),
    "dip_bn_bwd_apply_src_fin": (C.c_int, [C.POINTER(DipGradSrc), C.c_void_p, C.c_int, C.c_int, C.c_int, C.c_int, C.c_void_p,
                                           C.c_int, C.c_float, C.c_void_p, C.c_int, C.c_void_p, C.c_void_p, C.c_void_p,
                                           C.c_void_p, C.c_int, C.c_void_p]),
    "dip_bn_bwd_one_ok": (C.c_int, [C.c_int, C.c_int]),
    "dip_bn_bwd_one": (C.c_int, [C.POINTER(DipGradSrc), C.c_void_p, C.c_int, C.c_int, C.c_int, C.c_int, C.c_void_p, C.c_int,
                                 C.c_float, C.c_void_p, C.c_int, C.c_void_p, C.c_void_p, C.c_void_p, C.c_void_p]),
    "dip_upsample_bwd_one": (C.c_int, [C.c_void_p, C.c_int, C.c_int, C.c_int, C.c_int, C.c_int, C.c_int, C.c_int, C.c_int,
                                       C.c_int, C.c_void_p, C.c_int, C.c_int, C.c_void_p, C.c_int, C.c_float, C.c_void_p,
                                       C.c_int, C.c_void_p, C.c_void_p, C.c_void_p, C.c_void_p]),
    "dip_fold_to_nchw": (C.c_int, [C.POINTER(DipGradSrc), C.c_int, C.c_int, C.c_int, C.c_void_p, C.c_void_p]),
    "dip_fold_to_nhwc": (C.c_int, [C.POINTER(DipGradSrc), C.c_int, C.c_int, C.c_int, C.c_void_p, C.c_int, C.c_void_p]),
    "dip_res_join_fwd": (C.c_int, [C.c_void_p, C.c_int, C.POINTER(DipTransform), C.c_void_p, C.c_int, C.POINTER(DipTransform),
                                   C.c_void_p, C.c_int, C.c_int, C.c_int, C.c_void_p]),
    "dip_res_join_bwd": (C.c_int, [C.c_void_p, C.c_int, C.POINTER(DipGradSrc), C.c_void_p, C.c_int, C.POINTER(DipTransform),
                                   C.c_void_p, C.c_int, C.c_int, C.c_int, C.c_int, C.c_void_p]),
    "dip_upcat_fwd": (C.c_int, [C.POINTER(DipUpcatDesc), C.c_void_p]),
    "dip_upcat_nblk": (C.c_int, [C.c_int, C.c_int, C.c_int]),
    "dip_upcat_fwd_fin": (C.c_int, [C.POINTER(DipUpcatDesc), C.POINTER(DipBnFin), C.c_void_p]),
    "dip_fin_rows_ok": (C.c_int, [C.c_int, C.c_int]),
    "dip_bn_bwd_stats_fin": (C.c_int, [C.POINTER(DipGradSrc), C.c_void_p, C.c_int, C.c_int, C.c_int, C.c_int,
                                       C.c_void_p, C.c_int, C.c_float, C.c_void_p, C.c_int, C.c_void_p, C.c_int,
                                       C.POINTER(DipBnbFin), C.c_void_p]),
    "dip_upsample_bwd_stats_crop_fin": (C.c_int, [C.c_void_p, C.c_int, C.c_int, C.c_int, C.c_int, C.c_int, C.c_int,
                                                  C.c_int, C.c_int, C.c_int, C.c_void_p, C.c_int, C.c_int, C.c_void_p,
                                                  C.c_int, C.c_float, C.c_void_p, C.c_int, C.c_void_p, C.c_int,
                                                  C.POINTER(DipBnbFin), C.c_void_p]),
    "dip_avgpool2_fwd": (C.c_int, [C.c_void_p, C.c_int, C.c_int, C.c_int, C.c_int, C.c_void_p, C.c_int, C.c_void_p,
                                   C.c_int, C.c_void_p]),
    "dip_avgpool2_bwd": (C.c_int, [C.c_void_p, C.c_int, C.c_int, C.c_int, C.c_int, C.c_void_p, C.c_int, C.c_void_p]),
    "dip_maxpool2_fwd": (C.c_int, [C.c_void_p, C.c_int, C.c_int, C.c_int, C.c_int, C.c_void_p, C.c_int, C.c_void_p,
                                   C.c_int, C.c_void_p]),
    "dip_maxpool2_bwd": (C.c_int, [C.c_void_p, C.c_void_p, C.c_int, C.c_int, C.c_int, C.c_int, C.c_int, C.c_void_p,
                                   C.c_int, C.c_void_p]),
    "dip_upsample_bwd_stats": (C.c_int, [C.c_void_p, C.c_int, C.c_int, C.c_int, C.c_int, C.c_int, C.c_void_p,
                                         C.c_int, C.c_int, C.c_void_p, C.c_int, C.c_float, C.c_void_p, C.c_int,
                                         C.c_void_p, C.c_int, C.c_void_p]),
    "dip_upsample_bwd_stats_crop": (C.c_int, [C.c_void_p, C.c_int, C.c_int, C.c_int, C.c_int, C.c_int, C.c_int, C.c_int,
                                              C.c_int, C.c_int, C.c_void_p, C.c_int, C.c_int, C.c_void_p, C.c_int,
                                              C.c_float, C.c_void_p, C.c_int, C.c_void_p, C.c_int, C.c_void_p]),
    "dip_adam_step": (C.c_int, [C.c_void_p, C.c_void_p, C.c_void_p, C.c_void_p, C.c_int64, C.c_double, C.c_double,
                                C.c_double, C.c_double, C.c_int, C.c_void_p]),
    "dip_noise_axpy": (C.c_int, [C.c_void_p, C.c_void_p, C.c_int64, C.c_float, C.c_uint64, C.c_uint64, C.c_void_p]),
    "dip_adam_tick": (C.c_int, [C.c_void_p, C.c_double, C.c_double, C.c_double, C.c_void_p]),
    "dip_adam_step_dev": (C.c_int, [C.c_void_p, C.c_void_p, C.c_void_p, C.c_void_p, C.c_int64, C.c_double, C.c_double,
                                    C.c_double, C.c_void_p, C.c_void_p]),
    "dip_noise_axpy_dev": (C.c_int, [C.c_void_p, C.c_void_p, C.c_int64, C.c_float, C.c_uint64, C.c_void_p, C.c_void_p]),
    "dip_noise_axpy_dev2": (C.c_int, [C.c_void_p, C.c_void_p, C.c_int64, C.c_float, C.c_void_p, C.c_void_p]),
    "dip_counter_add": (C.c_int, [C.c_void_p, C.c_uint64, C.c_void_p]),
    "dip_counter_add_n": (C.c_int, [C.c_void_p, C.c_int, C.c_uint64, C.c_void_p]),
    "dip_group_begin": (C.c_int, [C.c_int, C.c_longlong, C.c_void_p, C.c_longlong]),
    "dip_group_end": (C.c_int, []),
    "dip_group_size": (C.c_int, []),
    "dip_group_native": (C.c_int, [C.c_int]),
    "dip_loss_head_nblk": (C.c_int, [C.c_int, C.c_int]),
    "dip_loss_head_fwd": (C.c_int, [C.POINTER(DipLossHeadDesc), C.c_void_p]),
    "dip_loss_head_bwd": (C.c_int, [C.POINTER(DipLossHeadDesc), C.c_void_p, C.c_void_p, C.c_int, C.c_void_p]),
    "dip_fit_monitor_nblk": (C.c_int, [C.c_int64]),
    "dip_fit_monitor": (C.c_int, [C.c_void_p, C.c_void_p, C.c_void_p, C.c_void_p, C.c_int64, C.c_float, C.c_int,
                                  C.c_void_p, C.c_void_p, C.c_void_p, C.c_void_p, C.c_int, C.c_float, C.c_void_p]),
    "dip_fit_monitor_dev": (C.c_int, [C.POINTER(DipFitMonitorDesc), C.c_void_p]),
    "dip_arena_backtrack": (C.c_int, [C.c_void_p, C.c_void_p, C.c_int64, C.c_void_p, C.c_void_p]),
    "dip_lanczos_down_fwd": (C.c_int, [C.c_void_p, C.c_void_p, C.c_void_p, C.c_int, C.c_int, C.c_int, C.c_int,
                                       C.c_int, C.c_int, C.c_void_p]),
    "dip_lanczos_down_bwd": (C.c_int, [C.c_void_p, C.c_void_p, C.c_void_p, C.c_int, C.c_int, C.c_int, C.c_int,
                                       C.c_int, C.c_int, C.c_void_p]),
    "dip_down_dense_fwd": (C.c_int, [C.c_void_p, C.c_void_p, C.c_void_p, C.c_void_p, C.c_int, C.c_int, C.c_int, C.c_int,
                                     C.c_int, C.c_int, C.c_void_p]),
    "dip_down_dense_bwd_data": (C.c_int, [C.c_void_p, C.c_void_p, C.c_void_p, C.c_int, C.c_int, C.c_int, C.c_int,
                                          C.c_int, C.c_int, C.c_void_p]),
    "dip_down_dense_bwd_weight": (C.c_int, [C.c_void_p, C.c_void_p, C.c_void_p, C.c_void_p, C.c_int, C.c_int, C.c_int,
                                            C.c_int, C.c_int, C.c_int, C.c_void_p]),
}

EXPORTS = tuple(_SIGS.keys())
_lib = None


def lib():
    global _lib
    if _lib is None:
        if not os.path.exists(LIB_PATH):
            raise RuntimeError(
                f"{LIB_PATH} is missing: the deep-image-prior MI355X backend has no fallback path. "
                "Build it with `python __graft_entry__.py build` (needs hipcc, targets gfx950).")
        L = C.CDLL(LIB_PATH)
        for name, (res, args) in _SIGS.items():
            fn = getattr(L, name)
            fn.restype = res
            fn.argtypes = args
        if L.dip_abi_version() != ABI_VERSION:
            raise RuntimeError(f"libdip_hip.so ABI {L.dip_abi_version()} != binding ABI {ABI_VERSION}")
        _lib = L
    return _lib


def check(rc: int, what: str = ""):
    if rc != 0:
        msg = lib().dip_last_error()
        raise RuntimeError(f"libdip_hip {what} failed (rc={rc}): {msg.decode() if msg else ''}")


def round_up(x: int, m: int) -> int:
    return (x + m - 1) // m * m


def conv_plan(Hout, Wout, Cin, Cout, ks, stride):
    k, rows, wsf = C.c_int(), C.c_int(), C.c_int64()
    check(lib().dip_conv_plan(Hout, Wout, Cin, Cout, ks, stride, C.byref(k), C.byref(rows), C.byref(wsf)), "conv_plan")
    return k.value, rows.value, wsf.value


def conv_plan_fp32(Hout, Wout, Cin, Cout, ks, stride):
    k, rows, wsf = C.c_int(), C.c_int(), C.c_int64()
    check(lib().dip_conv_plan_fp32(Hout, Wout, Cin, Cout, ks, stride, C.byref(k), C.byref(rows), C.byref(wsf)), "conv_plan_fp32")
    return k.value, rows.value, wsf.value


def conv_plan_dil2(Hout, Wout, Cin, Cout, ks):
    k, rows, wsf = C.c_int(), C.c_int(), C.c_int64()
    check(lib().dip_conv_plan_dil2(Hout, Wout, Cin, Cout, ks, C.byref(k), C.byref(rows), C.byref(wsf)), "conv_plan_dil2")
    return k.value, rows.value, wsf.value


def wgrad_plan(Hout, Wout, Cin, Cout, ks, stride):
    n = C.c_int()
    check(lib().dip_wgrad_plan(Hout, Wout, Cin, Cout, ks, stride, C.byref(n)), "wgrad_plan")
    return n.value


def wgrad_plan2(Hout, Wout, Cin, Cout, ks, stride):
    n, g, cb = C.c_int(), C.c_int(), C.c_int()
    check(lib().dip_wgrad_plan2(Hout, Wout, Cin, Cout, ks, stride, C.byref(n), C.byref(g), C.byref(cb)), "wgrad_plan2")
    return n.value, g.value, cb.value


CMD_LAUNCH, CMD_RECORD, CMD_WAIT = 0, 1, 2
_INT_TYPES = (C.c_int, C.c_int32, C.c_int64, C.c_longlong, C.c_uint64, C.c_uint32, C.c_long, C.c_ulong)


def _slot(argtype, v) -> int:
    import struct
    if argtype in _INT_TYPES:
        return int(v) & 0xFFFFFFFFFFFFFFFF
    if argtype is C.c_float:
        return int.from_bytes(struct.pack("<f", float(v)), "little")
    if argtype is C.c_double:
        return int.from_bytes(struct.pack("<d", float(v)), "little")
    if v is None:
        return 0
    if isinstance(v, int):
        return v & 0xFFFFFFFFFFFFFFFF
    obj = getattr(v, "_obj", None)
    if obj is not None:
        return C.addressof(obj)
    if isinstance(v, (C.c_void_p, C.c_char_p)):
        return int(v.value or 0)
    return C.addressof(v)


class CmdList:

    def __init__(self, cmds):
        L = lib()
        self.names = []
        self._keep = []
        n = len(cmds)
        self.arr = (DipCmd * max(n, 1))()
        self.nevents = 0
        for i, c in enumerate(cmds):
            if c[0] == "launch":
                _, fn, args, st, name = c
                fname = fn.__name__
                fid = L.dip_list_fn_id(fname.encode())
                if fid < 0:
                    raise RuntimeError(f"dip-amd: {fname} is not a command-list entry point")
                argtypes = _SIGS[fname][1]
                if len(args) + 1 != len(argtypes) or L.dip_list_fn_nargs(fid) != len(argtypes):
                    raise RuntimeError(f"dip-amd: {fname}: {len(args)} arguments for {len(argtypes) - 1} parameters")
                slots = (C.c_uint64 * len(argtypes))()
                for k, (t, v) in enumerate(zip(argtypes[:-1], args)):
                    slots[k] = _slot(t, v)
                self._keep.append((slots, args))
                self.arr[i] = DipCmd(CMD_LAUNCH, fid, st, -1, C.cast(slots, C.POINTER(C.c_uint64)), len(argtypes), 0)
                self.names.append(name)
            elif c[0] == "record":
                self.arr[i] = DipCmd(CMD_RECORD, -1, c[2], c[1], None, 0, 0)
                self.nevents = max(self.nevents, c[1] + 1)
                self.names.append("record")
            else:
                self.arr[i] = DipCmd(CMD_WAIT, -1, c[1], c[2], None, 0, 0)
                self.nevents = max(self.nevents, c[2] + 1)
                self.names.append("wait")
        self.n = n
        self._events = {}
        self._failed = C.c_int(-1)

    def _event_set(self, key):
        ev = self._events.get(key)
        if ev is None:
            ev = (C.c_void_p * max(self.nevents, 1))()
            if self.nevents:
                check(lib().dip_events_create(ev, self.nevents), "events_create")
            self._events[key] = ev
        return ev

    def run(self, stream_ptrs, key="eager"):
        ns = len(stream_ptrs)
        st = (C.c_void_p * ns)(*stream_ptrs)
        ev = self._event_set(key)
        rc = lib().dip_list_run(self.arr, self.n, st, ns, ev, self.nevents, C.byref(self._failed))
        if rc:
            k = self._failed.value
            check(rc, self.names[k] if 0 <= k < self.n else "list_run")

    def __del__(self):
        try:
            for ev in self._events.values():
                if self.nevents:
                    lib().dip_events_destroy(ev, self.nevents)
        except Exception:
            pass


class IterList:

    def __init__(self, phases, key="eager"):
        self.phases = list(phases)
        self.arr = (DipPhase * max(len(self.phases), 1))()
        for i, cl in enumerate(self.phases):
            ev = cl._event_set(key)
            self.arr[i] = DipPhase(C.cast(cl.arr, C.POINTER(DipCmd)), C.cast(ev, C.POINTER(C.c_void_p)), cl.n, cl.nevents)
        self.n = len(self.phases)
        self._failed = (C.c_int * 2)(-1, -1)
        self._streams = None
        self._stream_key = None
        self._run = lib().dip_iter_run

    def run(self, stream_ptrs):
        if stream_ptrs != self._stream_key:
            self._streams = (C.c_void_p * len(stream_ptrs))(*stream_ptrs)
            self._stream_key = list(stream_ptrs)
        rc = self._run(self.arr, self.n, self._streams, len(stream_ptrs), self._failed)
        if rc:
            p, k = self._failed[0], self._failed[1]
            name = "iter_run"
            if 0 <= p < self.n:
                names = self.phases[p].names
                name = f"phase {p}: " + (names[k] if 0 <= k < len(names) else "list_run")
            check(rc, name)
```

include/dip_hip.h:

```cpp
#ifndef DIP_HIP_H
#define DIP_HIP_H

#include <stdint.h>

#ifdef __cplusplus
extern "C" {
#endif

#define DIP_ABI_VERSION 8

#define DIP_PAD_ZERO 0
#define DIP_PAD_REFLECT 1
#define DIP_PAD_REPLICATE 2

#define DIP_ACT_SWISH (-1.0f)
#define DIP_ACT_ELU (-2.0f)
#define DIP_ACT_RELU (-3.0f)

#define DIP_UP_NEAREST 0
#define DIP_UP_BILINEAR 1

int dip_abi_version(void);
const char* dip_build_id(void);
const char* dip_last_error(void);
int dip_device_pci_bus_id(int device, char* buf, int len);


#define DIP_CMD_LAUNCH 0
#define DIP_CMD_RECORD 1
#define DIP_CMD_WAIT 2
typedef struct DipCmd {
    int32_t kind, fn, stream, event;
    uint64_t* slots;
    int32_t nslots, reserved;
} DipCmd;
int dip_list_fn_id(const char* name);
int dip_list_fn_nargs(int fn);
int dip_list_run(const DipCmd* cmds, int n, void* const* streams, int nstreams, void* const* events, int nevents,
                 int* failed_at);
int dip_events_create(void** events, int n);
int dip_events_destroy(void** events, int n);

typedef struct DipPhase {
    const DipCmd* cmds;
    void* const* events;
    int32_t n, nevents;
} DipPhase;
int dip_iter_run(const DipPhase* phases, int nphases, void* const* streams, int nstreams, int* failed_at);

int dip_group_begin(int ninst, long long stride_bytes, const void* base, long long row_bytes);
int dip_group_end(void);
int dip_group_size(void);
int dip_group_native(int mask);

typedef struct DipTransform {
    const float* a;
    const float* b;
    float slope;
} DipTransform;

int dip_nchw_to_nhwc(const float* src, float* dst, int C, int HW, int Cs, void* stream);
int dip_nhwc_to_nchw(const float* src, float* dst, int C, int HW, int Cs, int accumulate, void* stream);
int dip_head_fwd(const float* y, float* out, int C, int HW, int Cs, int sigmoid, void* stream);
int dip_head_bwd(const float* gout, const float* out, float* dy, int C, int HW, int Cs, int sigmoid,
                 void* stream);

typedef struct DipPackRec {
    int64_t w_off;
    int64_t fwd_off;
    int64_t dgrad_off;
    int32_t Cout, Cin, KS;
    int32_t CinP4, CoutP32, CoutP4, CinP32;
} DipPackRec;
int dip_pack_weights(const float* params, float* packed, const DipPackRec* recs_dev, int nrec,
                     int max_elems, void* stream);
typedef struct DipPackRec3 {
    int64_t w_off;
    int64_t fwd_off;
    int64_t dgrad_off;
    int32_t Cout, Cin, KS;
    int32_t nchF, CoutP32, nchD, CinP32;
} DipPackRec3;
int dip_pack_weights_bf3(const float* params, void* packed3, const DipPackRec3* recs_dev, int nrec, long long max_elems,
                         void* stream);

typedef struct DipBnFin {
    const float* gamma;
    const float* beta;
    float eps, momentum;
    float* state;
    int32_t Cs, C;
    float* running_mean;
    float* running_var;
    uint32_t* ticket;
} DipBnFin;
typedef struct DipBnbFin {
    float* dgamma;
    float* dbeta;
    float* coef;
    int32_t C, npix;
    uint32_t* ticket;
} DipBnbFin;

typedef struct DipConvDesc {
    const float* x;
    int32_t Hin, Win, Cx, Cin;
    DipTransform tr;
    const float* wp;
    const float* bias;
    float* y;
    int32_t Hout, Wout, Cy, Cout;
    int32_t y_pitch;
    int32_t ks, stride, pad_mode, off, dil, accumulate;
    float* stats;
    int32_t ksplit;
    float* ws;
    const float* bnb_y;
    const float* bnb_state;
    float* bnb_partials;
    float* bnb_partials_thin;
    int32_t bnb_Cy, bnb_Cs, bnb_pad;
    float bnb_slope;
    const void* wp3;
} DipConvDesc;
int dip_conv_igemm(const DipConvDesc* d, void* stream);
int dip_conv_ntiles(int Hout, int Wout);
int dip_conv_thin4_ntiles(int Hout, int Wout);
int dip_conv_bnb_fusable(const DipConvDesc* d);
int dip_conv_plan(int Hout, int Wout, int Cin, int Cout, int ks, int stride, int* ksplit, int* stats_rows,
                  int64_t* ws_floats);
int dip_conv_plan_fp32(int Hout, int Wout, int Cin, int Cout, int ks, int stride, int* ksplit, int* stats_rows,
                       int64_t* ws_floats);
int dip_conv_plan_dil2(int Hout, int Wout, int Cin, int Cout, int ks, int* ksplit, int* stats_rows,
                       int64_t* ws_floats);
int dip_conv_variant(const DipConvDesc* d);
int dip_conv_thin4(const DipConvDesc* d, int ncols, void* stream);
int dip_conv_igemm_dma_cols(const DipConvDesc* d, int n_base, void* stream);
int dip_conv_thin(const DipConvDesc* d, void* stream);
int dip_conv_thin_eligible(const DipConvDesc* d);
int dip_conv_thin_shape_ok(int Hout, int Wout, int Cin, int Cout, int ks, int stride);
int dip_conv_small(const DipConvDesc* d, void* stream);
int dip_conv_small_eligible(const DipConvDesc* d);
int dip_conv_small_rows(const DipConvDesc* d);
int dip_conv_dgrad_ring(const DipConvDesc* d, void* stream);
int dip_conv_dgrad_ring_ok(const DipConvDesc* d);
int dip_conv_bf3_eligible(const DipConvDesc* d);
int dip_conv_bf3_cols(const DipConvDesc* d, int n_base, int ncols, void* stream);
int dip_conv_bf3_terms(void);
int dip_conv_bf3_set_terms(int terms);
int dip_conv_splitk_finish(const DipConvDesc* d, void* stream);

typedef struct DipWgradDesc {
    const float* x;
    int32_t Hin, Win, Cx, Cin;
    DipTransform tr;
    const float* dy;
    int32_t Hout, Wout, Cdy, Cout;
    int32_t ks, stride, pad_mode, off;
    float* partial;
    float* bias_partial;
    int32_t nsplit;
    int32_t tap_groups;
    int32_t chan_block;
} DipWgradDesc;
int dip_conv_wgrad(const DipWgradDesc* d, void* stream);
int dip_wgrad_bf3_eligible(const DipWgradDesc* d);
int dip_wgrad_bf3(const DipWgradDesc* d, void* stream);
int dip_conv_wgrad_tail(const DipWgradDesc* d, void* stream);
int dip_wgrad_tail_stream_ok(const DipWgradDesc* d);
int dip_wgrad_tail_stream(const DipWgradDesc* d, void* stream);
int dip_wgrad_thin(const DipWgradDesc* d, void* stream);
int dip_wgrad_thin_eligible(const DipWgradDesc* d);
int dip_wgrad_thin_shape_ok(int Hout, int Wout, int Cin, int Cout, int ks, int stride);
int dip_wgrad_thin_nsplit(int Hout, int Wout, int Cin, int Cout, int ks, int stride);
int dip_conv_wgrad_ntiles(int Hout, int Wout);
int dip_wgrad_plan(int Hout, int Wout, int Cin, int Cout, int ks, int stride, int* nsplit);
int dip_wgrad_plan2(int Hout, int Wout, int Cin, int Cout, int ks, int stride, int* nsplit, int* tap_groups,
                    int* chan_block);
int dip_wgrad_reduce(const float* partial, const float* bias_partial, int nsplit, int ks, int Cin,
                     int Cout, float* dw , float* dbias , void* stream);

int dip_bn_finalize(const float* partials, int ntiles, int Cstride, int C, const float* gamma,
                    const float* beta, float eps, float momentum, float* state, int Cs,
                    float* running_mean, float* running_var, void* stream);

typedef struct DipGradSrc {
    const float* g;
    int32_t pad, fold, Cg, choff;
    int32_t win_y, win_x, win_h, win_w;
    const float* tw;
    int32_t tn, tcw;
} DipGradSrc;

int dip_bn_bwd_stats(const DipGradSrc* src, const float* y, int H, int W, int Cy, int C,
                     const float* state, int Cs, float slope, float* dz, int Cdz,
                     float* partials , int nblk, void* stream);
int dip_bn_bwd_nblk(int H, int W, int C);
int dip_bn_bwd_stats_fin(const DipGradSrc* src, const float* y, int H, int W, int Cy, int C,
                         const float* state, int Cs, float slope, float* dz, int Cdz,
                         float* partials , int nblk, const DipBnbFin* fin, void* stream);
int dip_bn_bwd_finalize(const float* partials, int nblk, int Cs, int C, int npix, float* dgamma,
                        float* dbeta, float* coef, void* stream);
int dip_bn_bwd_finalize2(const float* partials, int nblk, const float* partials_lo, int nblk_lo, int c_lo, int Cs,
                         int C, int npix, float* dgamma, float* dbeta, float* coef, void* stream);
int dip_bn_bwd_apply(float* dz, int Cdz, const float* y, int Cy, int npix, int C, const float* state,
                     int Cs, const float* coef, void* stream);
int dip_bn_bwd_apply_src(const DipGradSrc* src, const float* y, int H, int W, int Cy, int C,
                         const float* state, int Cs, float slope, const float* coef, float* dy, int Cdy,
                         void* stream);
int dip_bn_bwd_fin_rows_ok(int nrows, int C);
int dip_bn_bwd_apply_fin(float* dz, int Cdz, const float* y, int Cy, int npix, int C, const float* state, int Cs,
                         const float* partials, int nrows, float* dgamma, float* dbeta, float* coef, void* stream);
int dip_bn_bwd_apply_src_fin(const DipGradSrc* src, const float* y, int H, int W, int Cy, int C, const float* state, int Cs,
                             float slope, const float* partials, int nrows, float* dgamma, float* dbeta, float* coef,
                             float* dy, int Cdy, void* stream);
int dip_bn_bwd_one_ok(int npix, int C);
int dip_bn_bwd_one(const DipGradSrc* src, const float* y, int H, int W, int Cy, int C, const float* state, int Cs,
                   float slope, float* dy, int Cdy, float* dgamma, float* dbeta, float* coef, void* stream);
int dip_fold_to_nchw(const DipGradSrc* src, int H, int W, int C, float* dst, void* stream);
int dip_fold_to_nhwc(const DipGradSrc* src, int H, int W, int C, float* dst, int Cd, void* stream);

int dip_res_join_fwd(const float* xa, int Cxa, const DipTransform* ta, const float* xb, int Cxb, const DipTransform* tb,
                     float* out, int Co, int npix, int C, void* stream);
int dip_res_join_bwd(const float* g, int Cg, const DipGradSrc* src, const float* y, int Cy, const DipTransform* ty,
                     float* gout, int Cgo, int H, int W, int C, void* stream);

typedef struct DipUpcatDesc {
    const float* s; int32_t Cs_s, ns; DipTransform ts;
    const float* d; int32_t Cs_d, nd; DipTransform td;
    int32_t H, W, mode;
    float* cat; int32_t Cs_cat;
    float* stats; int32_t nblk;
    int32_t Hs, Ws, os_y, os_x;
    int32_t Hd, Wd, od_y, od_x;
} DipUpcatDesc;
int dip_upcat_fwd(const DipUpcatDesc* d, void* stream);
int dip_upcat_fwd_fin(const DipUpcatDesc* d, const DipBnFin* fin, void* stream);
int dip_fin_rows_ok(int rows, int C);
int dip_upcat_nblk(int H, int W, int C);

int dip_avgpool2_fwd(const float* x, int H, int W, int Cx, int C, float* y, int Cy, float* stats, int nblk,
                     void* stream);
int dip_avgpool2_bwd(const float* dy, int H, int W, int Cdy, int C, float* dx, int Cdx, void* stream);
int dip_maxpool2_fwd(const float* x, int H, int W, int Cx, int C, float* y, int Cy, float* stats, int nblk,
                     void* stream);
int dip_maxpool2_bwd(const float* dy, const float* x, int H, int W, int Cdy, int Cx, int C, float* dx, int Cdx,
                     void* stream);

int dip_upsample_bwd_stats(const float* dcat, int Cs_cat, int choff, int H, int W, int mode,
                           const float* y, int Cy, int C, const float* state, int Cs, float slope,
                           float* dz, int Cdz, float* partials, int nblk, void* stream);
int dip_upsample_bwd_stats_crop(const float* dcat, int Cs_cat, int choff, int H, int W, int Hd, int Wd, int od_y,
                                int od_x, int mode, const float* y, int Cy, int C, const float* state, int Cs,
                                float slope, float* dz, int Cdz, float* partials, int nblk, void* stream);

int dip_upsample_bwd_stats_crop_fin(const float* dcat, int Cs_cat, int choff, int H, int W, int Hd, int Wd, int od_y,
                                    int od_x, int mode, const float* y, int Cy, int C, const float* state, int Cs,
                                    float slope, float* dz, int Cdz, float* partials, int nblk, const DipBnbFin* fin,
                                    void* stream);

int dip_upsample_bwd_one(const float* dcat, int Cs_cat, int choff, int H, int W, int Hd, int Wd, int od_y, int od_x,
                         int mode, const float* y, int Cy, int C, const float* state, int Cs, float slope, float* dy,
                         int Cdy, float* dgamma, float* dbeta, float* coef, void* stream);

int dip_adam_step(float* p, const float* g, float* m, float* v, int64_t n, double lr, double beta1,
                  double beta2, double eps, int step, void* stream);

int dip_noise_axpy(const float* z, float* out, int64_t n, float sigma, uint64_t seed, uint64_t offset,
                   void* stream);

typedef struct DipIterState {
    uint64_t step;
    float step_size;
    float bc2_sqrt;
} DipIterState;
int dip_adam_tick(DipIterState* st, double lr, double beta1, double beta2, void* stream);
int dip_adam_step_dev(float* p, const float* g, float* m, float* v, int64_t n, double beta1, double beta2,
                      double eps, const DipIterState* st, void* stream);
int dip_noise_axpy_dev(const float* z, float* out, int64_t n, float sigma, uint64_t seed, uint64_t* offset_dev,
                       void* stream);
int dip_noise_axpy_dev2(const float* z, float* out, int64_t n, float sigma, uint64_t* state_dev, void* stream);
int dip_counter_add(uint64_t* counter, uint64_t inc, void* stream);
int dip_counter_add_n(uint64_t* counters, int n, uint64_t inc, void* stream);

typedef struct DipLossHeadDesc {
    const float* u;
    int Cu, Cin;
    DipTransform tr;
    const float* w;
    const float* bias;
    int Cout, HW, sigmoid;
    const float* target;
    const float* mask;
    int mask_c;
    float* out;
    float* partials;
    int nblk;
    float* loss;
} DipLossHeadDesc;
int dip_loss_head_nblk(int HW, int Cin);
int dip_loss_head_fwd(const DipLossHeadDesc* d, void* stream);
int dip_loss_head_bwd(const DipLossHeadDesc* d, const float* gscale, float* dy, int Cy, void* stream);

int dip_fit_monitor_nblk(int64_t n);
int dip_fit_monitor(const float* out, const float* noisy, const float* gt, float* out_avg, int64_t n,
                    float exp_weight, int first, const float* loss, float* partial, float* record,
                    float* state, int check_backtrack, float backtrack_db, void* stream);
typedef struct DipFitMonitorDesc {
    const float* out;
    const float* noisy;
    const float* gt;
    float* out_avg;
    int64_t n;
    float exp_weight, backtrack_db;
    const float* loss;
    float* partial;
    float* records;
    int capacity, show_every;
    int backtracking;
    int reserved;
    int* counter;
    float* state;
} DipFitMonitorDesc;
int dip_fit_monitor_dev(const DipFitMonitorDesc* d, void* stream);
int dip_arena_backtrack(float* params, float* snapshot, int64_t n, const float* state, void* stream);

int dip_lanczos_down_fwd(const float* x, const float* taps, float* y, int C, int H, int W, int k,
                         int factor, int pad, void* stream);
int dip_lanczos_down_bwd(const float* gy, const float* taps, float* gx, int C, int H, int W, int k,
                         int factor, int pad, void* stream);
int dip_down_dense_fwd(const float* x, const float* w, const float* bias, float* y, int C, int H, int W, int k,
                       int factor, int pad, void* stream);
int dip_down_dense_bwd_data(const float* gy, const float* w, float* gx, int C, int H, int W, int k, int factor,
                            int pad, void* stream);
int dip_down_dense_bwd_weight(const float* gy, const float* x, float* dw, float* db, int C, int H, int W, int k,
                              int factor, int pad, void* stream);

#ifdef __cplusplus
}
#endif
#endif
```

Baseline: 186.5.

## Fuse up-path 1x1 conv backward with BN-act backward and weight-gradient accumulation

Adds a persistent HIP kernel that, per 64-pixel tile, applies the pending BN/activation backward of the following layer, runs the 1x1 conv data-gradient with MFMA, accumulates BN statistics for the preceding BN, and optionally computes per-block weight and bias gradient partials. The engine defers the BN apply step as a pending gradient and routes the up-path 1x1 conv through this kernel by default. The aim is to remove several separate launches and intermediate round trips through global memory for dy, the gradient and the activations. The cost is a complex kernel with extra reduction passes over partials and new scheduling dependencies.

```diff
diff --git a/__graft_entry__.py b/__graft_entry__.py
--- a/__graft_entry__.py
+++ b/__graft_entry__.py
@@ -6,7 +6,7 @@
 PKG = os.path.join(ROOT, "deep-image-prior_amd")
 CSRC = os.path.join(PKG, "csrc")
 LIB = os.path.join(PKG, "lib", "libdip_hip.so")
-SOURCES = ["dip_core.hip", "dip_list.hip", "conv_igemm.hip", "conv_igemm_dma.hip", "conv_small.hip", "conv_thin.hip", "conv_bf3.hip", "conv1x1_res.hip", "conv_thin4.hip", "conv_wgrad.hip", "wgrad_bf3.hip", "wgrad_tail.hip", "wgrad_thin.hip", "bn_kernels.hip", "bn_bwd_one.hip",
+SOURCES = ["dip_core.hip", "dip_list.hip", "conv_igemm.hip", "conv_igemm_dma.hip", "conv_small.hip", "conv_thin.hip", "conv_bf3.hip", "conv1x1_res.hip", "conv1x1_bwd.hip", "conv_thin4.hip", "conv_wgrad.hip", "wgrad_bf3.hip", "wgrad_tail.hip", "wgrad_thin.hip", "bn_kernels.hip", "bn_bwd_one.hip",
            "upcat_kernels.hip", "res_kernels.hip", "misc_kernels.hip", "monitor_kernels.hip", "loss_kernels.hip"]
 
 
diff --git a/deep-image-prior_amd/csrc/conv1x1_bwd.hip b/deep-image-prior_amd/csrc/conv1x1_bwd.hip
--- /dev/null
+++ b/deep-image-prior_amd/csrc/conv1x1_bwd.hip
@@ -0,0 +1,282 @@
+#include "dip_common.h"
+#include "dip_group.h"
+#include "dip_gradsrc.h"
+#include <stdlib.h>
+
+template <class F> __host__ __device__ inline void dip_ptrs(Dip1x1BwdDesc& d, F& f) {
+    dip_ptrs(d.src, f);
+    f(d.y1); f(d.state1); f(d.coef1); f(d.dy1); f(d.w); f(d.y0); f(d.state0); f(d.g); f(d.partials); f(d.wpartial);
+    f(d.bias_partial);
+}
+
+namespace {
+
+constexpr int F_TP = 64;
+constexpr int F_C = 128;
+constexpr int F_NT = 512;
+constexpr int F_NI = F_TP / (F_NT / 32);
+constexpr int F_TILE = F_TP * F_C;
+constexpr int F_CST = 10 * F_C;
+constexpr int F_LDS_BYTES = (2 * F_TILE + F_CST) * 4;
+
+template <bool WG, bool GRP>
+__global__ __launch_bounds__(F_NT) void conv1x1_bwd_fused_kernel(const Dip1x1BwdDesc d_, const int ntiles,
+                                                                  const DipGrpArg<GRP> grp) {
+    DIP_GRP_DESC(Dip1x1BwdDesc, d);
+    extern __shared__ __attribute__((aligned(16))) float smem[];
+    float* dyS = smem;
+    float* xS = smem + F_TILE;
+    float* cst = smem + 2 * F_TILE;
+    const int tid = threadIdx.x;
+    const int lane = tid & 63;
+    const int wave = __builtin_amdgcn_readfirstlane(tid >> 6);
+    const int l31 = lane & 31, half = lane >> 5;
+    const int cb = wave & 3, ph = wave >> 2;
+    const int n = cb * 32 + l31;
+    const bool nv = n < d.Cin;
+    const bool wact = cb * 32 < d.Cin;
+    const int P = d.H * d.W;
+    const int Ci = d.Cin, Co = d.Cout;
+
+    for (int i = tid; i < F_CST; i += F_NT) {
+        const int row = i >> 7, c = i & 127;
+        float v = 0.f;
+        if (c < Co) {
+            if (row < 4) v = d.state1[row * d.Cs1 + c];
+            else if (row < 6) v = d.coef1[(row - 4) * d.Cs1 + c];
+            else if (d.src.tw != nullptr && row - 6 < d.src.tn) v = d.src.tw[(size_t)(row - 6) * d.src.tcw + c];
+        }
+        cst[i] = v;
+    }
+
+    const int nn = nv ? n : 0;
+    f32x4 wb[16];
+#pragma unroll
+    for (int kk = 0; kk < 16; ++kk)
+#pragma unroll
+        for (int j = 0; j < 4; ++j) {
+            const int o = 4 * (2 * kk + half) + j;
+            wb[kk][j] = d.w[min(o, Co - 1) * Ci + nn] * ((nv && o < Co) ? 1.f : 0.f);
+        }
+    const float m0 = d.state0[nn], r0 = d.state0[d.Cs0 + nn], a0 = d.state0[2 * d.Cs0 + nn], b0 = d.state0[3 * d.Cs0 + nn];
+    const float slope0 = d.slope0, slope1 = d.slope1;
+
+    const int cg = tid & 31, prow = tid >> 5;
+    const bool lact = cg * 4 < Co;
+    const int ch = lact ? cg * 4 : 0;
+    const int smode = d.src.tw != nullptr ? 0 : 1;
+    f32x4 yv[F_NI], gv[F_NI];
+    auto prefetch = [&](int tile) {
+        const int pbase = tile * F_TP + prow;
+#pragma unroll
+        for (int i = 0; i < F_NI; ++i) yv[i] = ld4(d.y1 + (size_t)min(pbase + 16 * i, P - 1) * d.Cy1 + ch);
+        if (smode == 0) {
+#pragma unroll
+            for (int i = 0; i < F_NI; ++i) gv[i] = ld4(d.src.g + (size_t)min(pbase + 16 * i, P - 1) * d.src.Cg);
+        } else {
+#pragma unroll
+            for (int i = 0; i < F_NI; ++i) gv[i] = ld4(d.src.g + d.src.choff + ch + (size_t)min(pbase + 16 * i, P - 1) * d.src.Cg);
+        }
+    };
+
+    f32x16 dw[2];
+    if constexpr (WG) {
+#pragma unroll
+        for (int j = 0; j < 2; ++j)
+#pragma unroll
+            for (int r = 0; r < 16; ++r) dw[j][r] = 0.f;
+    }
+    f32x4 bsum = f32x4{0.f, 0.f, 0.f, 0.f};
+    float g1 = 0.f, g2 = 0.f;
+
+    int tile = blockIdx.x;
+    prefetch(tile);
+    __syncthreads();
+    for (; tile < ntiles; tile += gridDim.x) {
+        {
+            const f32x4 mean = ld4(cst + ch), rstd = ld4(cst + F_C + ch), a = ld4(cst + 2 * F_C + ch),
+                        b = ld4(cst + 3 * F_C + ch), k1 = ld4(cst + 4 * F_C + ch), k2 = ld4(cst + 5 * F_C + ch);
+            GradSrcThin tw;
+#pragma unroll
+            for (int j = 0; j < 4; ++j) tw.w[j] = ld4(cst + (6 + j) * F_C + ch);
+#pragma unroll
+            for (int i = 0; i < F_NI; ++i) {
+                const int pl = prow + 16 * i;
+                const int p = tile * F_TP + pl;
+                const f32x4 du = smode == 0 ? grad_src_thin_du(d.src, tw, gv[i]) : gv[i];
+                const bool ok = lact && p < P;
+                f32x4 o;
+#pragma unroll
+                for (int e = 0; e < 4; ++e) {
+                    const float z = fmaf(a[e], yv[i][e], b[e]);
+                    const float gm = d.src_masked ? du[e] : dip_mul_rn(du[e], dip_act_grad(z, slope1));
+                    const float xh = (yv[i][e] - mean[e]) * rstd[e];
+                    o[e] = ok ? a[e] * (gm - k1[e] - xh * k2[e]) : 0.f;
+                }
+                st4(dyS + pl * F_C + ((cg ^ (pl & 7)) << 2), o);
+                if (ok && d.dy1 != nullptr) st4(d.dy1 + (size_t)p * d.Cdy1 + ch, o);
+                bsum += o;
+            }
+        }
+        __syncthreads();
+        {
+            const int next = tile + (int)gridDim.x;
+            if (next < ntiles) prefetch(next);
+        }
+        __builtin_amdgcn_sched_barrier(0);
+
+        f32x16 acc;
+#pragma unroll
+        for (int r = 0; r < 16; ++r) acc[r] = 0.f;
+        if (wact) {
+            const int px = 32 * ph + l31;
+            const float* arow = dyS + px * F_C;
+            const int sw = px & 7;
+            f32x4 fa = ld4(arow + ((half ^ sw) << 2)), fn = fa;
+#pragma unroll
+            for (int kk = 0; kk < 16; ++kk) {
+                if (kk < 15) fn = ld4(arow + (((2 * kk + 2 + half) ^ sw) << 2));
+#pragma unroll
+                for (int j = 0; j < 4; ++j) acc = __builtin_amdgcn_mfma_f32_32x32x2f32(fa[j], wb[kk][j], acc, 0, 0, 0);
+                fa = fn;
+            }
+        }
+
+        {
+            const int pl0 = 32 * ph + 4 * half;
+            const int p0 = tile * F_TP + pl0;
+            float y0v[16];
+#pragma unroll
+            for (int r = 0; r < 16; ++r)
+                y0v[r] = d.y0[(size_t)min(p0 + (r & 3) + 8 * (r >> 2), P - 1) * d.Cy0 + nn];
+#pragma unroll
+            for (int r = 0; r < 16; ++r) {
+                const int q = (r & 3) + 8 * (r >> 2);
+                if (nv && p0 + q < P) d.g[(size_t)(p0 + q) * d.Cg + n] = acc[r];
+            }
+#pragma unroll
+            for (int r = 0; r < 16; ++r) {
+                const int q = (r & 3) + 8 * (r >> 2);
+                const float z = fmaf(a0, y0v[r], b0);
+                const float gm = dip_mul_rn(acc[r], dip_act_grad(z, slope0));
+                g1 += gm;
+                g2 = fmaf(gm, (y0v[r] - m0) * r0, g2);
+                if constexpr (WG) xS[(pl0 + q) * F_C + n] = nv ? dip_act(z, slope0) : 0.f;
+            }
+        }
+
+        if constexpr (WG) {
+            __syncthreads();
+            if (wact) {
+                const int o0 = 32 * (2 * ph) + l31, o1 = o0 + 32;
+                const float* xa = xS + half * F_C + n;
+#pragma unroll 8
+                for (int s = 0; s < F_TP / 2; ++s) {
+                    const int pl = 2 * s + half;
+                    const float av = xa[2 * s * F_C];
+                    const float* drow = dyS + pl * F_C;
+                    const float bv0 = drow[(((o0 >> 2) ^ (pl & 7)) << 2) + (o0 & 3)];
+                    const float bv1 = drow[(((o1 >> 2) ^ (pl & 7)) << 2) + (o1 & 3)];
+                    dw[0] = __builtin_amdgcn_mfma_f32_32x32x2f32(av, bv0, dw[0], 0, 0, 0);
+                    dw[1] = __builtin_amdgcn_mfma_f32_32x32x2f32(av, bv1, dw[1], 0, 0, 0);
+                }
+            }
+        }
+        __syncthreads();
+    }
+
+    g1 += __shfl_xor(g1, 32);
+    g2 += __shfl_xor(g2, 32);
+    float* red = dyS;
+    float* redb = dyS + 4 * F_C;
+    if (half == 0) {
+        red[(ph * 2) * F_C + n] = g1;
+        red[(ph * 2 + 1) * F_C + n] = g2;
+    }
+    st4(redb + (prow * 32 + cg) * 4, lact ? bsum : f32x4{0.f, 0.f, 0.f, 0.f});
+    __syncthreads();
+    if (tid < d.Cs0 && tid < F_C) {
+        float* o = d.partials + (size_t)blockIdx.x * 2 * d.Cs0 + tid;
+        o[0] = tid < Ci ? red[tid] + red[2 * F_C + tid] : 0.f;
+        o[d.Cs0] = tid < Ci ? red[F_C + tid] + red[3 * F_C + tid] : 0.f;
+    }
+    if constexpr (WG) {
+        const int CoutP = (Co + 31) & ~31, CinP = (Ci + 31) & ~31;
+        if (d.bias_partial != nullptr && tid < CoutP) {
+            float s = 0.f;
+#pragma unroll
+            for (int r = 0; r < F_NT / 32; ++r) s += redb[(r * 32 + (tid >> 2)) * 4 + (tid & 3)];
+            d.bias_partial[(size_t)blockIdx.x * CoutP + tid] = s;
+        }
+        float* slab = d.wpartial + (size_t)blockIdx.x * CinP * CoutP;
+#pragma unroll
+        for (int j = 0; j < 2; ++j) {
+            const int ob = 2 * ph + j;
+            if (32 * cb < CinP && 32 * ob < CoutP) {
+#pragma unroll
+                for (int r = 0; r < 16; ++r) {
+                    const int c = 32 * cb + (r & 3) + 8 * (r >> 2) + 4 * half;
+                    slab[(size_t)c * CoutP + 32 * ob + l31] = dw[j][r];
+                }
+            }
+        }
+    }
+}
+
+int device_cus() {
+    static int ncus[16] = {};
+    int dev = 0;
+    if (hipGetDevice(&dev) != hipSuccess || dev < 0 || dev >= 16) dev = 0;
+    if (ncus[dev] == 0) {
+        hipDeviceProp_t prop;
+        if (hipGetDeviceProperties(&prop, dev) == hipSuccess) ncus[dev] = prop.multiProcessorCount;
+        if (ncus[dev] <= 0) ncus[dev] = 256;
+    }
+    return ncus[dev];
+}
+
+}
+
+extern "C" int dip_conv1x1_bwd_rows(int npix) {
+    const int ntiles = dip_cdiv(npix, F_TP);
+    const int ncu = device_cus();
+    return ntiles < ncu ? ntiles : ncu;
+}
+
+extern "C" int dip_conv1x1_bwd_fused(const Dip1x1BwdDesc* dp, void* stream) {
+    const Dip1x1BwdDesc& d = *dp;
+    if (d.Cin < 4 || d.Cout < 4 || d.Cin > F_C || d.Cout > F_C || (d.Cin & 3) || (d.Cout & 3))
+        DIP_FAIL("conv1x1_bwd_fused: Cin, Cout must be multiples of 4 in 4..128");
+    if (d.H < 1 || d.W < 1 || (long long)d.H * d.W > (1ll << 30)) DIP_FAIL("conv1x1_bwd_fused: image size");
+    if ((d.Cy1 & 3) || (d.Cs1 & 3) || (d.Cdy1 & 3) || (d.Cy0 & 3) || (d.Cs0 & 3) || (d.Cg & 3) || (d.src.Cg & 3) || (d.src.choff & 3))
+        DIP_FAIL("conv1x1_bwd_fused: channel strides must be multiples of 4");
+    if (d.Cy1 < d.Cout || d.Cs1 < d.Cout || d.Cy0 < d.Cin || d.Cs0 < d.Cin || d.Cg < d.Cin || (d.dy1 != nullptr && d.Cdy1 < d.Cout))
+        DIP_FAIL("conv1x1_bwd_fused: a channel stride is smaller than its channel count");
+    if (d.src.g == nullptr || d.y1 == nullptr || d.state1 == nullptr || d.coef1 == nullptr || d.w == nullptr || d.y0 == nullptr ||
+        d.state0 == nullptr || d.g == nullptr || d.partials == nullptr)
+        DIP_FAIL("conv1x1_bwd_fused: a required pointer is NULL");
+    if (d.src.tw != nullptr && (d.src.tn < 1 || d.src.tn > 4 || d.src.tcw < d.Cout || d.src.Cg < 4))
+        DIP_FAIL("conv1x1_bwd_fused: thin source needs 1..4 rows of >= Cout weights");
+    if (d.src.tw == nullptr && (d.src.pad != 0 || d.src.fold != 0 || d.src.win_h > 0))
+        DIP_FAIL("conv1x1_bwd_fused: the gradient source must be a thin conv or a plain [H][W][Cg] tensor (no pad / fold / window)");
+    if (d.src.tw == nullptr && d.src.Cg < d.src.choff + d.Cout) DIP_FAIL("conv1x1_bwd_fused: the gradient source has fewer channels than Cout");
+    if (d.wpartial == nullptr && d.bias_partial != nullptr) DIP_FAIL("conv1x1_bwd_fused: bias_partial without wpartial");
+    const int ntiles = dip_cdiv(d.H * d.W, F_TP);
+    if (d.nrows < 1 || d.nrows > ntiles) DIP_FAIL("conv1x1_bwd_fused: nrows must be in 1..ceil(H*W/64) (dip_conv1x1_bwd_rows)");
+    static bool attr_set[16] = {};
+    if (dip_once_per_device(attr_set)) {
+        hipError_t e = dip_pair_lds_attr(conv1x1_bwd_fused_kernel<false, false>, conv1x1_bwd_fused_kernel<false, true>, F_LDS_BYTES);
+        if (e == hipSuccess)
+            e = dip_pair_lds_attr(conv1x1_bwd_fused_kernel<true, false>, conv1x1_bwd_fused_kernel<true, true>, F_LDS_BYTES);
+        if (e != hipSuccess) { dip_set_error(hipGetErrorString(e)); return (int)e; }
+    }
+    hipStream_t st = reinterpret_cast<hipStream_t>(stream);
+    if (d.wpartial != nullptr)
+        dip_launch_pair<DIP_FAM_CONV>(conv1x1_bwd_fused_kernel<true, false>, conv1x1_bwd_fused_kernel<true, true>, dim3(d.nrows),
+                                      dim3(F_NT), F_LDS_BYTES, st, d, ntiles);
+    else
+        dip_launch_pair<DIP_FAM_CONV>(conv1x1_bwd_fused_kernel<false, false>, conv1x1_bwd_fused_kernel<false, true>, dim3(d.nrows),
+                                      dim3(F_NT), F_LDS_BYTES, st, d, ntiles);
+    DIP_CHECK_LAUNCH();
+    return 0;
+}
diff --git a/deep-image-prior_amd/csrc/dip_gradsrc.h b/deep-image-prior_amd/csrc/dip_gradsrc.h
--- a/deep-image-prior_amd/csrc/dip_gradsrc.h
+++ b/deep-image-prior_amd/csrc/dip_gradsrc.h
@@ -13,14 +13,16 @@
     for (int j = 0; j < 4; ++j) t.w[j] = (s.tw != nullptr && j < s.tn) ? ld4(s.tw + (size_t)j * s.tcw + ch) : f32x4{0.f, 0.f, 0.f, 0.f};
     return t;
 }
-__device__ __forceinline__ f32x4 grad_src_thin4(const DipGradSrc& s, const GradSrcThin& t, int r, int c, int W) {
-    f32x4 gv = ld4(s.g + ((size_t)r * W + c) * s.Cg);
+__device__ __forceinline__ f32x4 grad_src_thin_du(const DipGradSrc& s, const GradSrcThin& t, f32x4 gv) {
 #pragma unroll
     for (int j = 1; j < 4; ++j) gv[j] = j < s.tn ? gv[j] : 0.f;
     f32x4 du;
 #pragma unroll
     for (int e = 0; e < 4; ++e) du[e] = fmaf(gv[3], t.w[3][e], fmaf(gv[2], t.w[2][e], fmaf(gv[1], t.w[1][e], gv[0] * t.w[0][e])));
     return du;
+}
+__device__ __forceinline__ f32x4 grad_src_thin4(const DipGradSrc& s, const GradSrcThin& t, int r, int c, int W) {
+    return grad_src_thin_du(s, t, ld4(s.g + ((size_t)r * W + c) * s.Cg));
 }
 
 __device__ __forceinline__ f32x4 grad_src4(const DipGradSrc& s, int r, int c, int H, int W, int ch) {
diff --git a/deep-image-prior_amd/csrc/dip_list.hip b/deep-image-prior_amd/csrc/dip_list.hip
--- a/deep-image-prior_amd/csrc/dip_list.hip
+++ b/deep-image-prior_amd/csrc/dip_list.hip
@@ -43,7 +43,7 @@
     DIP_REG(dip_noise_axpy_dev), DIP_REG(dip_noise_axpy_dev2), DIP_REG(dip_counter_add), DIP_REG(dip_counter_add_n),
     DIP_REG(dip_loss_head_fwd), DIP_REG(dip_loss_head_bwd), DIP_REG(dip_fit_monitor), DIP_REG(dip_fit_monitor_dev), DIP_REG(dip_arena_backtrack),
     DIP_REG(dip_lanczos_down_fwd), DIP_REG(dip_lanczos_down_bwd), DIP_REG(dip_down_dense_fwd), DIP_REG(dip_down_dense_bwd_data),
-    DIP_REG(dip_down_dense_bwd_weight), DIP_REG(dip_res_join_fwd), DIP_REG(dip_res_join_bwd),
+    DIP_REG(dip_down_dense_bwd_weight), DIP_REG(dip_res_join_fwd), DIP_REG(dip_res_join_bwd), DIP_REG(dip_conv1x1_bwd_fused),
 };
 constexpr int NFN = (int)(sizeof(g_fns) / sizeof(g_fns[0]));
 
diff --git a/deep-image-prior_amd/dip_engine.py b/deep-image-prior_amd/dip_engine.py
--- a/deep-image-prior_amd/dip_engine.py
+++ b/deep-image-prior_amd/dip_engine.py
@@ -8,6 +8,8 @@
 
 import dip_native as N
 from dip_native import round_up
+
+UP1_FUSE_DEFAULT = 1
 
 
 def _ptr(t: Optional[torch.Tensor], off_floats: int = 0) -> Optional[int]:
@@ -65,6 +67,12 @@
             return N.DipTransform(1, 1, self.slope)
         assert self.bn.Cs == self.Cs
         return N.DipTransform(_ptr(self.bn.state, 2 * self.Cs), _ptr(self.bn.state, 3 * self.Cs), self.slope)
+
+
+class _PendingDy:
+
+    def __init__(self, src, masked, dz):
+        self.src, self.masked, self.dz = src, masked, dz
 
 
 class ScalePlan:
@@ -108,7 +116,10 @@
         self._clists = {}
         self._replicate_bufs = set()
         self.fuse_bnb = os.environ.get("DIP_BNB_FUSE", "0") == "1"
-        self.fuse_bnb_1x1 = os.environ.get("DIP_BNB_FUSE", "0") == "2"
+        self.up1_fuse = int(os.environ.get("DIP_UP1_FUSE", str(UP1_FUSE_DEFAULT)))
+        if self.up1_fuse not in (0, 1, 2):
+            raise ValueError("DIP_UP1_FUSE must be 0, 1 or 2")
+        self.up1_fuse_min_pixels = int(os.environ.get("DIP_UP1_FUSE_MIN_PIXELS", "4625"))
         self.thin_src = os.environ.get("DIP_NO_THIN_SRC") is None
         self.use_small = os.environ.get("DIP_CONV_NO_SMALL") is None
         self.ticket_fin = os.environ.get("DIP_TICKET_FIN") == "1"
@@ -318,7 +329,7 @@
             else:
                 du_last = self._emit_dgrad(oc, last, self.dy_out, pre, fuse_bn=True)
             dy_last = self._emit_bn_act_bwd(last, du_last, pre)
-            self.dbg_top = {"du_last": du_last, "dy_last": dy_last, "last": last}
+            self.dbg_top = {"du_last": du_last, "dy_last": dy_last.dz if isinstance(dy_last, _PendingDy) else dy_last, "last": last}
             self.last_act = last
             self.bwd_ops = pre + self._bwd_scale_ops(0, dy_last)
             self.bwd_ops += self._flush_deferred_wgrads()
@@ -343,6 +354,7 @@
             self._alloc.append(self.tickets)
         self._ticket_off = 0
         self._fused_bnb = {}
+        self._up1_fused = {}
         self._deferred = []
         self._replicate_bufs = set()
         self._fwd_side = set()
@@ -404,12 +416,22 @@
             self._emit_conv_fwd(s.up1, u, st["u1_y"], s.up1_bn)
             res = Act(st["u1_y"], Ho, Wo, s.up1.Cout, s.up1_bn, self.slope)
             st["u1"] = res
+            res.up1_fuse = self._up1_fuse_ok(s.up1, u, res)
         st["xin"], st["H"], st["W"], st["Ho"], st["Wo"] = xin, H, W, Ho, Wo
         s.st = st
         return res
 
     def _buf(self, n):
         return None if self._sizing else self._new(n)
+
+    def _up1_fuse_ok(self, r: ConvRec, x: Act, y: Act) -> bool:
+        if not self.up1_fuse or self.ticket_fin or self.bnb_fin_fuse:
+            return False
+        if r.ks != 1 or r.stride != 1 or r.P != 0 or r.Cin > 128 or r.Cout > 128 or r.Cin % 4 or r.Cout % 4:
+            return False
+        if x.bn is None or y.bn is None or x.H * x.W < self.up1_fuse_min_pixels:
+            return False
+        return not self._bnb_one_ok(x) and not self._bnb_one_ok(y)
 
     def _ticket(self, n=8):
         if self._sizing:
@@ -591,8 +613,7 @@
         if r.stride == 2:
             ksplit, _, wsf = N.conv_plan_dil2(Hg, Wg, round_up(r.Cout, 4), r.Cin, r.ks)
         else:
-            fuse_here = self.fuse_bnb or (self.fuse_bnb_1x1 and r.ks == 1 and r.stride == 1)
-            bf3_ok = self.bf3 and getattr(r, "dgrad3_off", -1) >= 0 and not (fuse_bn and fuse_here and not ring and x.bn is not None)
+            bf3_ok = self.bf3 and getattr(r, "dgrad3_off", -1) >= 0 and not (fuse_bn and self.fuse_bnb and not ring and x.bn is not None)
             ksplit, _, wsf = (N.conv_plan if bf3_ok else N.conv_plan_fp32)(Hg, Wg, round_up(r.Cout, 4), r.Cin, r.ks, 1)
         sizing = self._sizing
         d = N.DipConvDesc(None if sizing else _ptr(dy), Ho, Wo, round_up(r.Cout, 4), round_up(r.Cout, 4),
@@ -623,8 +644,7 @@
             return (gbuf, pad)
         variant = self.lib.dip_conv_variant(C.byref(d))
         fused = None
-        fuse_here = self.fuse_bnb or (self.fuse_bnb_1x1 and r.ks == 1 and r.stride == 1)
-        if fuse_bn and fuse_here and not ring and x.bn is not None and self.lib.dip_conv_bnb_fusable(C.byref(d)):
+        if fuse_bn and self.fuse_bnb and not ring and x.bn is not None and self.lib.dip_conv_bnb_fusable(C.byref(d)):
             bn = x.bn
             rows = self.lib.dip_conv_ntiles(Hg, Wg)
             c_lo = (r.Cin - 128) if variant == 3 else 0
@@ -659,6 +679,52 @@
             ops.append((self.lib.dip_conv_dgrad_ring, (C.byref(dr),), "dgring:" + r.name))
         return (gbuf, pad)
 
+    def _emit_up1_fused(self, i, pend, ops):
+        s = self.sc[i]
+        st = s.st
+        r, x, a1 = s.up1, st["u"], st["u1"]
+        bn0, bn1 = x.bn, a1.bn
+        npix = x.H * x.W
+        rows = self.lib.dip_conv1x1_bwd_rows(npix)
+        CinP, CoutP = round_up(r.Cin, 32), round_up(r.Cout, 32)
+        with_wg = self.up1_fuse == 2
+        has_b = r.b_off >= 0
+        slab = self._buf(rows * CinP * CoutP) if with_wg else None
+        bslab = self._buf(rows * CoutP) if (with_wg and has_b) else None
+        gbuf = self._buf(npix * x.Cs)
+        if self._sizing:
+            self.bwdp_need = max(self.bwdp_need, rows * 2 * bn0.Cs)
+            if not with_wg:
+                self._emit_wgrad(r, x, None, ops, scale=i)
+            return None
+        lib = self.lib
+        d = N.Dip1x1BwdDesc()
+        d.src = pend.src
+        d.y1, d.state1, d.coef1, d.dy1 = _ptr(a1.buf), _ptr(bn1.state), _ptr(bn1.coef), _ptr(pend.dz)
+        d.w, d.y0, d.state0, d.g = _ptr(self.params, r.w_off), _ptr(x.buf), _ptr(bn0.state), _ptr(gbuf)
+        d.partials, d.wpartial, d.bias_partial = _ptr(self.bwd_scratch), _ptr(slab), _ptr(bslab)
+        d.H, d.W, d.Cin, d.Cout = x.H, x.W, r.Cin, r.Cout
+        d.Cy1, d.Cs1, d.Cdy1, d.Cy0, d.Cs0, d.Cg = a1.Cs, bn1.Cs, a1.Cs, x.Cs, bn0.Cs, x.Cs
+        d.nrows, d.src_masked, d.slope1, d.slope0 = rows, pend.masked, float(a1.slope), float(x.slope)
+        self.keep.append(d)
+        fname = "bnb_apply:" + bn1.name
+        ops.append((lib.dip_conv1x1_bwd_fused, (C.byref(d),), fname))
+        self._up1_fused[fname] = "wgred:" + r.name
+        if with_wg:
+            tgt = self._deferred if self.defer_scale >= 0 else ops
+            tgt.append((lib.dip_wgrad_reduce, (_ptr(slab), _ptr(bslab), rows, 1, r.Cin, r.Cout, _ptr(self.grads, r.w_off),
+                                               _ptr(self.grads, r.b_off) if has_b else None), "wgred:" + r.name))
+        else:
+            self._emit_wgrad(r, x, pend.dz, ops, scale=i)
+        ops.append((lib.dip_bn_bwd_finalize2, (_ptr(self.bwd_scratch), rows, None, 0, 0, bn0.Cs, bn0.C, npix,
+                                               _ptr(self.grads, bn0.gamma_off), _ptr(self.grads, bn0.beta_off),
+                                               _ptr(bn0.coef)), "bnb_fin:" + bn0.name))
+        dz0 = self._new(npix * x.Cs)
+        src0 = self._gradsrc((gbuf, 0), x.Cs)
+        ops.append((lib.dip_bn_bwd_apply_src, (C.byref(src0), _ptr(x.buf), x.H, x.W, x.Cs, x.C, _ptr(bn0.state), bn0.Cs,
+                                               float(x.slope), _ptr(bn0.coef), _ptr(dz0), x.Cs), "bnb_apply:" + bn0.name))
+        return dz0
+
     def _thin_src_ok(self, oc: ConvRec, last: Act) -> bool:
         return (self.thin_src and oc.ks == 1 and oc.stride == 1 and oc.Cout <= 4 and oc.Cin % 4 == 0 and last.bn is not None
                 and not self.fuse_bnb and not self._bnb_one_ok(last))
@@ -683,13 +749,30 @@
         nblk = self.lib.dip_bn_bwd_nblk(a.H, a.W, a.C)
         fin_ok = self.ticket_fin and bool(self.lib.dip_fin_rows_ok(nblk, a.C))
         ticket = self._ticket() if fin_ok else None
+        pend = getattr(a, "up1_fuse", False) and not side and (len(g) == 3 or (g[1] == 0 and window is None))
         if self._sizing:
             if side:
                 self.bwdp2_need = max(self.bwdp2_need, nblk * 2 * a.Cs)
             else:
                 self.bwdp_need = max(self.bwdp_need, nblk * 2 * a.Cs)
-            return None
+            return _PendingDy(None, 0, None) if pend else None
         scratch = self.bwd_scratch2 if side else self.bwd_scratch
+        if pend:
+            src = self._gradsrc(g, Cg if Cg is not None else a.Cs, choff, window)
+            fused = self._fused_bnb.get(g[0].data_ptr()) if choff == 0 else None
+            if fused is not None:
+                rows, rows_lo, c_lo = fused
+                ops.append((self.lib.dip_bn_bwd_finalize2, (_ptr(self.bwd_scratch), rows, _ptr(self.bwd_scratch3) if c_lo else None,
+                                                            rows_lo, c_lo, bn.Cs, bn.C, a.H * a.W,
+                                                            _ptr(self.grads, bn.gamma_off), _ptr(self.grads, bn.beta_off),
+                                                            _ptr(bn.coef)), "bnb_fin:" + bn.name))
+            else:
+                ops.append((self.lib.dip_bn_bwd_stats, (C.byref(src), _ptr(a.buf), a.H, a.W, a.Cs, a.C, _ptr(bn.state), bn.Cs,
+                                                        float(a.slope), None, a.Cs, _ptr(scratch), nblk), "bnb_stats:" + bn.name))
+                ops.append((self.lib.dip_bn_bwd_finalize, (_ptr(scratch), nblk, bn.Cs, bn.C, a.H * a.W,
+                                                           _ptr(self.grads, bn.gamma_off), _ptr(self.grads, bn.beta_off),
+                                                           _ptr(bn.coef)), "bnb_fin:" + bn.name))
+            return _PendingDy(src, 0, self._new(a.H * a.W * a.Cs) if self.up1_fuse == 1 else None)
         dz = self._new(a.H * a.W * a.Cs)
         src = self._gradsrc(g, Cg if Cg is not None else a.Cs, choff, window)
         lib = self.lib
@@ -745,9 +828,10 @@
         nblk = self.lib.dip_bn_bwd_nblk(deep.H, deep.W, deep.C)
         fin_ok = self.ticket_fin and bool(self.lib.dip_fin_rows_ok(nblk, deep.C))
         ticket = self._ticket() if fin_ok else None
+        pend = getattr(deep, "up1_fuse", False)
         if self._sizing:
             self.bwdp_need = max(self.bwdp_need, nblk * 2 * deep.Cs)
-            return None
+            return _PendingDy(None, 1, None) if pend else None
         dz = self._new(deep.H * deep.W * deep.Cs)
         lib = self.lib
         m = N.UP_BILINEAR if mode == "bilinear" else N.UP_NEAREST
@@ -778,6 +862,11 @@
                         (_ptr(dcat), Cs_cat, choff, H, W, geom["Hd"], geom["Wd"], geom["od_y"], geom["od_x"], m,
                          _ptr(deep.buf), deep.Cs, deep.C, _ptr(bn.state), bn.Cs, float(deep.slope), _ptr(dz), deep.Cs,
                          _ptr(self.bwd_scratch), nblk), "upb_stats:" + bn.name))
+        if pend:
+            ops.append((lib.dip_bn_bwd_finalize, (_ptr(self.bwd_scratch), nblk, bn.Cs, bn.C, deep.H * deep.W,
+                                                  _ptr(self.grads, bn.gamma_off), _ptr(self.grads, bn.beta_off),
+                                                  _ptr(bn.coef)), "bnb_fin:" + bn.name))
+            return _PendingDy(self._gradsrc((dz, 0), deep.Cs), 1, dz)
         if self._fin_rows_ok(nblk, deep.C):
             ops.append((lib.dip_bn_bwd_apply_fin, (_ptr(dz), deep.Cs, _ptr(deep.buf), deep.Cs, deep.H * deep.W, deep.C,
                                                    _ptr(bn.state), bn.Cs, _ptr(self.bwd_scratch), nblk,
@@ -800,7 +889,10 @@
             ops += self._flush_deferred_wgrads()
         H, W, xin = st["H"], st["W"], st["xin"]
         Ho, Wo, geom = st["Ho"], st["Wo"], st["geom"]
-        if s.up1 is not None:
+        if isinstance(dy_last, _PendingDy):
+            dy_u = self._emit_up1_fused(i, dy_last, ops)
+            dy_last = dy_last.dz
+        elif s.up1 is not None:
             self._emit_wgrad(s.up1, st["u"], dy_last, ops, scale=i)
             g = self._emit_dgrad(s.up1, st["u"], dy_last, ops, fuse_bn=True)
             dy_u = self._emit_bn_act_bwd(st["u"], g, ops)
@@ -976,6 +1068,9 @@
             c = f"wgrad:s{i}.skip_conv"
             if sc.ns and c in present and p in present:
                 deps.setdefault(c, []).append(p)
+        for name, red in self._up1_fused.items():
+            if name in present and red in present and "wgrad:" + red[len("wgred:"):] not in present:
+                deps.setdefault(red, []).append(name)
         for k, name in enumerate(names):
             if not name.startswith("dgthin:"):
                 continue
diff --git a/deep-image-prior_amd/dip_native.py b/deep-image-prior_amd/dip_native.py
--- a/deep-image-prior_amd/dip_native.py
+++ b/deep-image-prior_amd/dip_native.py
@@ -67,6 +67,16 @@
     _fields_ = [("g", C.c_void_p), ("pad", C.c_int32), ("fold", C.c_int32), ("Cg", C.c_int32), ("choff", C.c_int32),
                 ("win_y", C.c_int32), ("win_x", C.c_int32), ("win_h", C.c_int32), ("win_w", C.c_int32),
                 ("tw", C.c_void_p), ("tn", C.c_int32), ("tcw", C.c_int32)]
+
+
+class Dip1x1BwdDesc(C.Structure):
+    _fields_ = [("src", DipGradSrc), ("y1", C.c_void_p), ("state1", C.c_void_p), ("coef1", C.c_void_p), ("dy1", C.c_void_p),
+                ("w", C.c_void_p), ("y0", C.c_void_p), ("state0", C.c_void_p), ("g", C.c_void_p), ("partials", C.c_void_p),
+                ("wpartial", C.c_void_p), ("bias_partial", C.c_void_p),
+                ("H", C.c_int32), ("W", C.c_int32), ("Cin", C.c_int32), ("Cout", C.c_int32),
+                ("Cy1", C.c_int32), ("Cs1", C.c_int32), ("Cdy1", C.c_int32), ("Cy0", C.c_int32), ("Cs0", C.c_int32),
+                ("Cg", C.c_int32), ("nrows", C.c_int32), ("src_masked", C.c_int32),
+                ("slope1", C.c_float), ("slope0", C.c_float)]
 
 
 class DipUpcatDesc(C.Structure):
@@ -243,6 +253,8 @@
     "dip_fit_monitor": (C.c_int, [C.c_void_p, C.c_void_p, C.c_void_p, C.c_void_p, C.c_int64, C.c_float, C.c_int,
                                   C.c_void_p, C.c_void_p, C.c_void_p, C.c_void_p, C.c_int, C.c_float, C.c_void_p]),
     "dip_fit_monitor_dev": (C.c_int, [C.POINTER(DipFitMonitorDesc), C.c_void_p]),
+    "dip_conv1x1_bwd_rows": (C.c_int, [C.c_int]),
+    "dip_conv1x1_bwd_fused": (C.c_int, [C.POINTER(Dip1x1BwdDesc), C.c_void_p]),
     "dip_arena_backtrack": (C.c_int, [C.c_void_p, C.c_void_p, C.c_int64, C.c_void_p, C.c_void_p]),
     "dip_lanczos_down_fwd": (C.c_int, [C.c_void_p, C.c_void_p, C.c_void_p, C.c_int, C.c_int, C.c_int, C.c_int,
                                        C.c_int, C.c_int, C.c_void_p]),
diff --git a/include/dip_hip.h b/include/dip_hip.h
--- a/include/dip_hip.h
+++ b/include/dip_hip.h
@@ -220,6 +220,27 @@
 int dip_fold_to_nchw(const DipGradSrc* src, int H, int W, int C, float* dst, void* stream);
 int dip_fold_to_nhwc(const DipGradSrc* src, int H, int W, int C, float* dst, int Cd, void* stream);
 
+typedef struct Dip1x1BwdDesc {
+    DipGradSrc src;
+    const float* y1;
+    const float* state1;
+    const float* coef1;
+    float* dy1;
+    const float* w;
+    const float* y0;
+    const float* state0;
+    float* g;
+    float* partials;
+    float* wpartial;
+    float* bias_partial;
+    int32_t H, W, Cin, Cout;
+    int32_t Cy1, Cs1, Cdy1, Cy0, Cs0, Cg;
+    int32_t nrows, src_masked;
+    float slope1, slope0;
+} Dip1x1BwdDesc;
+int dip_conv1x1_bwd_rows(int npix);
+int dip_conv1x1_bwd_fused(const Dip1x1BwdDesc* d, void* stream);
+
 int dip_res_join_fwd(const float* xa, int Cxa, const DipTransform* ta, const float* xb, int Cxb, const DipTransform* tb,
                      float* out, int Co, int npix, int C, void* stream);
 int dip_res_join_bwd(const float* g, int Cg, const DipGradSrc* src, const float* y, int Cy, const DipTransform* ty,
```

Result: faster. 188.4, median of 6 (+1.0%).
